# orangeai-research/Generative-Multimodal-Recommendation

Hardware: AMD Instinct MI355X
Metric: train users/sec + full-rank eval users/sec, DiffMM Amazon-baby, 1/2/4/8 MI355X (higher is better)
Workload: dtype fp32; 1 GPU; DiffMM baby-shaped synthetic: 19445 users x 7050 items, 121517 train interactions; step = one DiffMMTrainer epoch (diffusion train + graph rebuild + BPR/contrastive); global_batch=2048, eval_batch=4096, parallelism=dp1

## Files before the change

### generative-multimodal-recommendation_amd/csrc/gemm.hip

```cpp
#include <stdlib.h>

#include <type_traits>

#include "gemm_impl.h"

namespace {
using namespace gmr_gemm;

template <int BM, int BN, int WGM, int WGN, bool AKC, bool BKC, bool VEC, int MF>
__global__ void __launch_bounds__(64 * WGM * WGN) gemm_kernel(int64_t M, int64_t N, int64_t K,
                                                             const float* __restrict__ A, int64_t lda,
                                                             const float* __restrict__ B, int64_t ldb,
                                                             float* __restrict__ C, int64_t ldc, Epi epi, int tiles_n,
                                                             int64_t k_per_split, float* __restrict__ ws) {
  constexpr int NT = 64 * WGM * WGN;
  constexpr int WTM = BM / WGM, WTN = BN / WGN;
  constexpr int TM = WTM / MF, TN = WTN / MF;
  using AccT = typename std::conditional<MF == 32, floatx16, floatx4>::type;
  constexpr int NE = MF == 32 ? 16 : 4;
  using SA = Stage<BM, AKC, VEC, NT>;
  using SB = Stage<BN, BKC, VEC, NT>;
  __shared__ __attribute__((aligned(16))) float smem[2 * (SA::WORDS + SB::WORDS)];
  constexpr int STAGE_WORDS = SA::WORDS + SB::WORDS;

// ... 444 lines not shown
  int64_t tm, tn, kps;
  int xpose;
  bool x6p;
};

int default_mfma() {
  static int mf = [] {
    const char* e = getenv("GMR_GEMM_MFMA");
    return (e && atoi(e) == 16) ? 16 : 32;
  }();
  return mf;
}

bool default_x6() {
  static bool x = [] {
    const char* e = getenv("GMR_GEMM_X6");
    return !(e && atoi(e) == 0);
  }();
  return x;
}

bool default_x6_64() {
  static bool x = [] {
    const char* e = getenv("GMR_GEMM_X6_64");
    return !(e && atoi(e) == 0);
  }();
  return x;
}

bool default_glds() {
  static bool g = [] {
    const char* e = getenv("GMR_GEMM_GLDS");
    return !(e && atoi(e) == 0);
  }();
  return g;
}

int auto_splits(int64_t tm, int64_t tn, int bm, int64_t K) {
  const bool skinny = bm == 64 && (tm == 1 || tn == 1);
  const int64_t min_k = skinny ? 192 : 512;
  const int max_s = skinny ? 64 : 16;
  int s = 1;
  while (tm * tn * s < 512 && K / (s * 2) >= min_k && s < max_s) s *= 2;
  if (bm == 128) {
    const int64_t slots = 512;
    auto waves = [&](int q) { return (double)(tm * tn * q) / (double)slots; };
    auto fill = [&](int q) {
      const int64_t w = tm * tn * q;
      return (double)w / (double)(((w + slots - 1) / slots) * slots);
    };
    while ((waves(s) < 8.0 || fill(s) < 0.9) && K / (s * 2) >= min_k && s < max_s) s *= 2;
  }
  return s;
}

Plan make_plan_core(int ta, int tb, int64_t M, int64_t N, int64_t K, int tile, int split_k, bool allow_x6) {
  int mf = default_mfma();
  if (tile & GMR_GEMM_MFMA16) mf = 16;
  if (tile & GMR_GEMM_MFMA32) mf = 32;
  bool glds = default_glds();
  if (tile & GMR_GEMM_GLDS) glds = true;
  if (tile & GMR_GEMM_REGSTAGE) glds = false;
  const bool x6 = allow_x6 && ((tile & GMR_GEMM_X6) || default_x6()) &&
                  !(tile & (GMR_GEMM_F32 | GMR_GEMM_MFMA16 | GMR_GEMM_MFMA32 | GMR_GEMM_GLDS | GMR_GEMM_REGSTAGE));
  const bool x6_64 = x6 && ((tile & GMR_GEMM_X6) || default_x6_64());
  const bool x6_pipe1 = tile & GMR_GEMM_X6_PIPE1;
  tile &= ~(GMR_GEMM_MFMA16 | GMR_GEMM_MFMA32 | GMR_GEMM_GLDS | GMR_GEMM_REGSTAGE | GMR_GEMM_X6 | GMR_GEMM_F32 |
            GMR_GEMM_X6_PIPE1);
  if (tile == 0) {
    const bool tnm = ta && !tb;
    auto fill = [](int64_t tiles, int64_t slots) { return (double)tiles / (double)(((tiles + slots - 1) / slots) * slots); };
    const bool wide256 = M >= 2048 && N >= 4096 && K >= 256 && K <= 1024 &&
                         fill(((M + 255) / 256) * ((N + 255) / 256), 256) >=
                             0.92 * fill(((M + 127) / 128) * ((N + 127) / 128), 512);
    auto score = [&](int t) {
      const int64_t tm = (M + t - 1) / t, tn = (N + t - 1) / t;
      const int s = auto_splits(tm, tn, t, K);
      double pen = 1.0;
      for (int q = s; q > 1; q >>= 1) pen *= 0.95;
      return fill(tm * tn * s, t == 256 ? 256 : 512) * pen * (t == 256 ? 1.03 : 1.0);
    };
    if (!tnm && M >= 2048 && N >= 1000 && K >= 4096)
      tile = (tb || !glds) && score(256) >= score(128) ? 256 : 128;
    else if (!tnm && wide256) tile = 256;
    else if (!tnm && M * N >= (int64_t)8 << 20 && K >= 512) tile = 128;
    else if (!tnm && M * N >= (int64_t)1 << 20 && K >= 4096) tile = 128;
    else if (!ta && !tb && N <= 64 && M >= 4096 && K >= 2048) tile = 12864;
    else tile = 64;
  }
  if (x6 && tile == 64 && M * N >= ((int64_t)4 << 20) && K >= 256) tile = 128;
  if (x6 && (tile != 64 || x6_64) && tile != 12864 && !ta && tb) {
    mf = 6;
    if (tile == 256) tile = ((M + 127) / 128) * ((N + 127) / 128) >= 768 ? 128 : 256128;
  }
  Plan p;
  p.mf = mf;
  p.glds = glds && mf == 32;
  p.tile = tile;
  p.bm = tile == 256128 ? 256 : tile == 128256 || tile == 12864 ? 128 : tile;
  p.bn = tile == 256128 ? 128 : tile == 128256 ? 256 : tile == 12864 ? 64 : tile;
  p.tm = (M + p.bm - 1) / p.bm;
  p.tn = (N + p.bn - 1) / p.bn;
  int splits = split_k;
  if (splits <= 0 && mf == 6) {
    static const int64_t min_slab_env = [] {
      const char* e = getenv("GMR_X6_MIN_SLAB");
      const int v = e ? atoi(e) : 0;
      return (int64_t)(v >= 64 ? v : 0);
    }();
    const int64_t min_slab = min_slab_env ? min_slab_env : p.bm == 64 ? (x6_ring() && K <= 1024 ? K : 256) : 512;
    const int64_t slots = p.bm == 64 ? 768 : p.bm * p.bn == 128 * 128 ? 512 : 256;
    splits = 1;
    while (p.tm * p.tn * splits * 5 < slots * 4 && K / (splits * 2) >= min_slab && splits < 16) splits *= 2;
  }
  if (splits <= 0) splits = auto_splits(p.tm, p.tn, p.bm, K);
  int64_t kps = (K + splits - 1) / splits;
  kps = (kps + BK - 1) / BK * BK;
  p.splits = (int)((K + kps - 1) / kps);
  p.kps = kps;
  p.xpose = 0;
  p.x6p = mf == 6 && x6_pipe1;
  return p;
}

Plan make_plan(int ta, int tb, int64_t M, int64_t N, int64_t K, int tile, int split_k) {
  if (ta || !tb) {
    Plan q = make_plan_core(0, 1, M, N, K, tile, split_k, true);
    if (q.mf == 6 && q.bm != 64) {
      q.xpose = (ta ? 1 : 0) | (tb ? 0 : 2);
      return q;
    }
    return make_plan_core(ta, tb, M, N, K, tile, split_k, false);
  }
  return make_plan_core(ta, tb, M, N, K, tile, split_k, true);
}

struct WsLayout {
  int64_t slabs, at, bt, total, kp;
};
WsLayout ws_layout(const Plan& p, int64_t M, int64_t N, int64_t K) {
  auto r4 = [](int64_t v) { return (v + 3) / 4 * 4; };
  WsLayout w;
  w.kp = r4(K);
  const bool uses = p.splits > 1 || p.xpose;
  w.slabs = GMR_GEMM_COUNTER_WORDS;
  w.at = uses ? r4(GMR_GEMM_COUNTER_WORDS + (p.splits > 1 ? (int64_t)p.splits * M * N : 0)) : 0;
  w.bt = w.at + ((p.xpose & 1) ? r4(M * w.kp) : 0);
  w.total = w.bt + ((p.xpose & 2) ? r4(N * w.kp) : 0);
  return w;
}

}

extern "C" int32_t gmr_gemm_kernel_kind(int32_t trans_a, int32_t trans_b, int64_t M, int64_t N, int64_t K,
                                        int32_t tile, int32_t split_k, int32_t aligned) {
  if (M <= 0 || N <= 0 || K <= 0) return 0;
  const Plan p = make_plan(trans_a, trans_b, M, N, K, tile, split_k);
  if (p.mf == 6 && !aligned && p.xpose != 3)
    return make_plan_core(trans_a, trans_b, M, N, K, tile, split_k, false).mf;
  return p.mf;
}

extern "C" int64_t gmr_gemm_workspace_floats(int32_t trans_a, int32_t trans_b, int64_t M, int64_t N, int64_t K,
                                             int32_t tile, int32_t split_k) {
  if (M <= 0 || N <= 0 || K <= 0) return 0;
  const Plan p = make_plan(trans_a, trans_b, M, N, K, tile, split_k);
  int64_t need = ws_layout(p, M, N, K).total;
  if (p.mf == 6) {
    const Plan q = make_plan_core(trans_a, trans_b, M, N, K, tile, split_k, false);
    need = std::max(need, ws_layout(q, M, N, K).total);
  }
  return need;
}

extern "C" int gmr_gemm_f32(int32_t trans_a, int32_t trans_b, int64_t M, int64_t N, int64_t K, float alpha,
                            const float* A, int64_t lda, const float* B, int64_t ldb, float beta, float* C,
                            int64_t ldc, int32_t epilogue, const float* bias, const int32_t* bias_row, int64_t ld_bias,
                            const float* aux, int64_t ld_aux, const float* rowvec1, const float* rowvec2, float slope,
                            int32_t tile, int32_t split_k, float* workspace, int64_t workspace_floats, void* stream) {
  GMR_ARG(A && B && C, "null operand");
  GMR_ARG(M > 0 && N > 0 && K > 0, "empty GEMM");
  GMR_ARG(lda >= (trans_a ? M : K) && ldb >= (trans_b ? K : N) && ldc >= N, "leading dimension too small");
  GMR_ARG(epilogue >= GMR_EPI_NONE && epilogue <= GMR_EPI_SCALE_BIAS, "bad epilogue");
  GMR_ARG(epilogue != GMR_EPI_LEAKY_NORM ||
              (N == 64 && aux && rowvec1 && ld_aux >= 64 && ld_aux % 4 == 0 && ldc % 4 == 0 &&
               (((uintptr_t)aux | (uintptr_t)C) & 15) == 0),
          "GMR_EPI_LEAKY_NORM: N = 64, 16-byte aligned C and aux (the normalised rows), rowvec1 (the norms)");
  GMR_ARG(!(epilogue == GMR_EPI_POSTERIOR || epilogue == GMR_EPI_DTANH || epilogue == GMR_EPI_ROWSCALE_AUX ||
            epilogue == GMR_EPI_DRELU) || aux,
          "epilogue needs aux");
  GMR_ARG(epilogue != GMR_EPI_ROWSCALE_AUX || rowvec1, "epilogue needs rowvec1");
  {
    const int t = tile & ~(GMR_GEMM_MFMA16 | GMR_GEMM_MFMA32 | GMR_GEMM_GLDS | GMR_GEMM_REGSTAGE | GMR_GEMM_X6 |
                           GMR_GEMM_F32 | GMR_GEMM_X6_PIPE1);
    GMR_ARG(t == 0 || t == 64 || t == 128 || t == 256 || t == 256128 || t == 128256 || t == 12864,
            "tile must be 0 (auto), 64, 128, 256, 256128, 128256 or 12864 (| GMR_GEMM_MFMA16 / GMR_GEMM_MFMA32)");
  }
  Epi e;
  e.kind = epilogue;
  e.alpha = alpha;
  e.beta = beta;
  e.slope = slope;
  e.bias = bias;
  e.bias_row = bias_row;
  e.ld_bias = ld_bias;
  e.aux = aux;
  e.ld_aux = ld_aux;
  e.rv1 = rowvec1;
  e.rv2 = rowvec2;
  const bool a16 = ((uintptr_t)A % 16 == 0) && lda % 4 == 0, b16 = ((uintptr_t)B % 16 == 0) && ldb % 4 == 0;
  bool vec = a16 && b16;
  Plan pl = make_plan(trans_a, trans_b, M, N, K, tile, split_k);
  if (pl.mf == 6 && !(((pl.xpose & 1) || a16) && ((pl.xpose & 2) || b16)))
    pl = make_plan_core(trans_a, trans_b, M, N, K, tile, split_k, false);
  if ((pl.xpose & 2) && x6_inplace()) pl.xpose &= ~2;
  if (pl.xpose == 1 && !trans_b && x6_inplace() == 2) pl.xpose = 0;
  const WsLayout wl = ws_layout(pl, M, N, K);
  if (pl.xpose) {
    GMR_ARG(workspace && workspace_floats >= wl.total, "needs workspace of gmr_gemm_workspace_floats(...) floats");
    GMR_ARG(((uintptr_t)workspace & 15) == 0, "workspace must be 16-byte aligned");
    if (pl.xpose & 1) {
      x6_transpose(A, lda, K, M, workspace + wl.at, wl.kp, (hipStream_t)stream);
      GMR_LAUNCHED();
      A = workspace + wl.at;
      lda = wl.kp;
    }
    if (pl.xpose & 2) {
      x6_transpose(B, ldb, K, N, workspace + wl.bt, wl.kp, (hipStream_t)stream);
      GMR_LAUNCHED();
      B = workspace + wl.bt;
      ldb = wl.kp;
    }
    if (pl.xpose & 1) trans_a = 0;
    if (pl.xpose & 2) trans_b = 1;
    vec = (pl.xpose & 1 ? true : a16) && (pl.xpose & 2 ? true : b16);
  }
  tile = pl.tile;
  const int64_t tm = pl.tm, tn = pl.tn, kps = pl.kps;
  const int splits = pl.splits;
  GMR_ARG(tm * tn < (1ll << 31), "too many tiles");
  float* ws = nullptr;
  int* counters = nullptr;
  if (splits > 1) {
    GMR_ARG(workspace && workspace_floats >= GMR_GEMM_COUNTER_WORDS + (int64_t)splits * M * N,
            "split-K needs workspace of gmr_gemm_workspace_floats(...) floats");
    ws = workspace + GMR_GEMM_COUNTER_WORDS;
    if (pl.glds && vec && tm * tn <= GMR_GEMM_COUNTER_WORDS && inkernel_fixup() && epilogue != GMR_EPI_LEAKY_NORM)
      counters = reinterpret_cast<int*>(workspace);
  }
  GMR_ARG(epilogue != GMR_EPI_LEAKY_NORM || splits > 1, "GMR_EPI_LEAKY_NORM needs a split-K plan");
  hipStream_t st = (hipStream_t)stream;
  dim3 grid((unsigned)(tm * tn), 1, (unsigned)splits);
  const int tnp = (int)tn | (tile_group(tn) << 20);
  int lrc = 0;
  switch (tile) {
    case 256:
      lrc = launch_tile<256, 256, 4, 4>(pl.mf, pl.glds, trans_a, trans_b, vec, grid, st, M, N, K, A, lda, B, ldb, C, ldc, e, tnp, kps, ws, counters, pl.x6p);
      break;
    case 256128:
      lrc = launch_tile<256, 128, 4, 2>(pl.mf, pl.glds, trans_a, trans_b, vec, grid, st, M, N, K, A, lda, B, ldb, C, ldc, e, tnp, kps, ws, counters, pl.x6p);
      break;
    case 128256:
      lrc = launch_tile<128, 256, 2, 4>(pl.mf, pl.glds, trans_a, trans_b, vec, grid, st, M, N, K, A, lda, B, ldb, C, ldc, e, tnp, kps, ws, counters, pl.x6p);
      break;
    case 12864:
      lrc = launch_tile<128, 64, 2, 2>(pl.mf, pl.glds, trans_a, trans_b, vec, grid, st, M, N, K, A, lda, B, ldb, C, ldc, e, tnp, kps, ws, counters, pl.x6p);
      break;
    case 128:
      lrc = launch_tile<128, 128, 2, 2>(pl.mf, pl.glds, trans_a, trans_b, vec, grid, st, M, N, K, A, lda, B, ldb, C, ldc, e, tnp, kps, ws, counters, pl.x6p);
      break;
    default:
      lrc = launch_tile<64, 64, 2, 2>(pl.mf, pl.glds, trans_a, trans_b, vec, grid, st, M, N, K, A, lda, B, ldb, C, ldc, e, tnp, kps, ws, counters, pl.x6p);
  }
  GMR_ARG(lrc == 0, "no split-bf16 kernel for this tile and operand layout");
  GMR_LAUNCHED();
  if (ws && !counters && epilogue == GMR_EPI_LEAKY_NORM) {
    hipLaunchKernelGGL(splitk_reduce_leaky_norm_kernel, dim3(gmr::grid_for(M * 16, 256)), dim3(256), 0, st, M, splits,
                       ws, C, ldc, e, const_cast<float*>(aux), ld_aux, const_cast<float*>(rowvec1));
    GMR_LAUNCHED();
  } else if (ws && !counters) {
    hipLaunchKernelGGL(splitk_reduce_kernel, dim3(gmr::grid_for(M * N, 256)), dim3(256), 0, st, M, N, splits, ws, C,
                       ldc, e);
    GMR_LAUNCHED();
  }
  return GMR_OK;
}
```

### generative-multimodal-recommendation_amd/csrc/gemm_impl.h

```cpp
#pragma once
#include <type_traits>

#include "gmr_common.h"

typedef float floatx16 __attribute__((ext_vector_type(16)));
typedef float floatx4 __attribute__((ext_vector_type(4)));

namespace gmr_gemm {

constexpr int BK = 32;

struct Epi {
  int kind;
  float alpha, beta, slope;
  const float* bias;
  const int* bias_row;
  int64_t ld_bias;
  const float* aux;
  int64_t ld_aux;
  const float* rv1;
  const float* rv2;
};

__device__ __forceinline__ bool epi_reads_x(const Epi& e) {
// ... 165 lines not shown
        const float b = epi.bias ? epi.bias[n] : 0.f;
#pragma unroll
        for (int e = 0; e < NE; ++e) {
          const int64_t m = m0 + wm * WTM + i * MF + (MF == 32 ? (e & 3) + 8 * (e >> 2) + 4 * h : 4 * h + e);
          if (m < M) C[m * ldc + n] = epi_fin(epi, acc[i][j][e], b, 0.f, 0.f, 0.f);
        }
      }
    return;
  }
#pragma unroll
  for (int i = 0; i < TM; ++i)
#pragma unroll
    for (int j = 0; j < TN; ++j) {
      const int64_t n = n0 + wn * WTN + j * MF + l32;
      if (n >= N) continue;
      float bv[NE], xv[NE];
#pragma unroll
      for (int e = 0; e < NE; ++e) {
        const int64_t m = m0 + wm * WTM + i * MF + (MF == 32 ? (e & 3) + 8 * (e >> 2) + 4 * h : 4 * h + e);
        const bool ok = m < M;
        bv[e] = (epi.bias && ok) ? epi.bias[(epi.bias_row ? (int64_t)epi.bias_row[m] : 0) * epi.ld_bias + n] : 0.f;
        xv[e] = (rx && ok) ? *epi_x_ptr(epi, C, ldc, m, n) : 0.f;
      }
#pragma unroll
      for (int e = 0; e < NE; ++e) {
        const int64_t m = m0 + wm * WTM + i * MF + (MF == 32 ? (e & 3) + 8 * (e >> 2) + 4 * h : 4 * h + e);
        if (m < M) C[m * ldc + n] = epi_fin(epi, acc[i][j][e], bv[e], xv[e], epi_r1(epi, m), epi_r2(epi, m));
      }
    }
}

__device__ __forceinline__ void tile_mn(int tile, int tn_packed, int tiles_m, int& tmi, int& tni) {
  const int tiles_n = tn_packed & 0xFFFFF, G = tn_packed >> 20;
  if (G <= 1) {
    tmi = tile / tiles_n;
    tni = tile - tmi * tiles_n;
    return;
  }
  const int per = G * tiles_n, g = tile / per, first = g * G;
  const int gs = min(tiles_m - first, G), rem = tile - g * per;
  tni = rem / gs;
  tmi = first + rem - tni * gs;
}


struct EpiCtx {
  const float* xb;
  int64_t ldx;
  bool rx, pure, v_in, v_out;
};
__device__ __forceinline__ EpiCtx epi_ctx(const Epi& epi, const float* C, int64_t ldc) {
  EpiCtx c;
  c.rx = epi_reads_x(epi);
  c.pure = !c.rx && !epi.bias_row && !epi.rv1 && !epi.rv2;
  c.xb = (epi.kind == GMR_EPI_NONE || epi.kind == GMR_EPI_BIAS) ? C : epi.aux;
  c.ldx = (epi.kind == GMR_EPI_NONE || epi.kind == GMR_EPI_BIAS) ? ldc : epi.ld_aux;
  c.v_out = ldc % 4 == 0 && ((uintptr_t)C & 15) == 0;
  c.v_in = (!epi.bias || (((uintptr_t)epi.bias & 15) == 0 && (!epi.bias_row || epi.ld_bias % 4 == 0))) &&
           (!c.rx || (((uintptr_t)c.xb & 15) == 0 && c.ldx % 4 == 0));
  return c;
}
__device__ __forceinline__ void epi_store4(const Epi& epi, float* __restrict__ C, int64_t ldc, int64_t N, int64_t m,
                                           int64_t n, const float (&a4)[4], const EpiCtx& ctx) {
  const bool full = n + 3 < N;
  float b4[4] = {0.f, 0.f, 0.f, 0.f}, x4[4] = {0.f, 0.f, 0.f, 0.f};
  const float* bp = epi.bias ? epi.bias + (epi.bias_row ? (int64_t)epi.bias_row[m] * epi.ld_bias : 0) + n : nullptr;
  const float* xp = ctx.rx ? ctx.xb + m * ctx.ldx + n : nullptr;
  if (full && ctx.v_in) {
    if (bp) {
      const float4 t = *reinterpret_cast<const float4*>(bp);
      b4[0] = t.x, b4[1] = t.y, b4[2] = t.z, b4[3] = t.w;
    }
    if (xp) {
      const float4 t = *reinterpret_cast<const float4*>(xp);
      x4[0] = t.x, x4[1] = t.y, x4[2] = t.z, x4[3] = t.w;
    }
  } else {
    for (int q = 0; q < 4 && n + q < N; ++q) {
      if (bp) b4[q] = bp[q];
      if (xp) x4[q] = xp[q];
    }
  }
  const float r1 = ctx.pure ? 0.f : epi_r1(epi, m), r2 = ctx.pure ? 0.f : epi_r2(epi, m);
  float o4[4];
#pragma unroll
  for (int q = 0; q < 4; ++q) o4[q] = epi_fin(epi, a4[q], b4[q], x4[q], r1, r2);
  float* o = C + m * ldc + n;
  if (full && ctx.v_out) {
    *reinterpret_cast<float4*>(o) = make_float4(o4[0], o4[1], o4[2], o4[3]);
  } else {
    for (int q = 0; q < 4 && n + q < N; ++q) o[q] = o4[q];
  }
}

template <int BM, int BN, int WGM, int WGN, int AVAIL = 2 * (BM + BN) * BK>
__device__ __forceinline__ void gemm_epilogue_lds(const floatx16 (&acc)[BM / WGM / 32][BN / WGN / 32], float* smem,
                                                  int64_t M, int64_t N, float* __restrict__ C, int64_t ldc,
                                                  const Epi& epi, int64_t m0, int64_t n0, float* __restrict__ ws) {
  constexpr int NT = 64 * WGM * WGN;
  constexpr int WTM = BM / WGM, WTN = BN / WGN;
  constexpr int TM = WTM / 32, TN = WTN / 32;
  constexpr int HR0 = (AVAIL / BN) / 32 * 32;
  constexpr int HR = HR0 < BM ? HR0 : BM;
  constexpr int C4 = BN / 4;
  const int lane = threadIdx.x & 63;
  const int w = threadIdx.x >> 6;
  const int wm = w / WGN, wn = w % WGN;
  const int h = lane >> 5, l32 = lane & 31;
  const EpiCtx ctx = epi_ctx(epi, C, ldc);
  const bool v_out = ws ? (N % 4 == 0 && ((uintptr_t)ws & 15) == 0) : ctx.v_out;
#pragma unroll
  for (int r0 = 0; r0 < BM; r0 += HR) {
    __syncthreads();
#pragma unroll
    for (int i = 0; i < TM; ++i) {
      const int rb = wm * WTM + i * 32;
      if (rb < r0 || rb >= r0 + HR) continue;
#pragma unroll
      for (int j = 0; j < TN; ++j) {
        const int col = wn * WTN + j * 32 + l32;
#pragma unroll
        for (int e = 0; e < 16; ++e) smem[(rb - r0 + (e & 3) + 8 * (e >> 2) + 4 * h) * BN + col] = acc[i][j][e];
      }
    }
    __syncthreads();
    const int rows = BM - r0 < HR ? BM - r0 : HR;
    for (int idx = threadIdx.x; idx < rows * C4; idx += NT) {
      const int rr = idx / C4, c = (idx % C4) * 4;
      const int64_t m = m0 + r0 + rr, n = n0 + c;
      if (m >= M || n >= N) continue;
      const float4 v = *reinterpret_cast<const float4*>(smem + rr * BN + c);
      const float a4[4] = {v.x, v.y, v.z, v.w};
      const bool full = n + 3 < N;
      if (ws) {
        float* o = ws + ((int64_t)blockIdx.z * M + m) * N + n;
        if (full && v_out) {
          *reinterpret_cast<float4*>(o) = v;
        } else {
          for (int q = 0; q < 4 && n + q < N; ++q) o[q] = a4[q];
        }
        continue;
      }
      epi_store4(epi, C, ldc, N, m, n, a4, ctx);
    }
  }
}

int x6_ring();
int x6_inplace();
int x6_launch(int bm, int bn, dim3 grid, hipStream_t st, int64_t M, int64_t N, int64_t K, const float* A, int64_t lda,
              const float* B, int64_t ldb, float* C, int64_t ldc, const Epi& epi, int tiles_n, int64_t kps, float* ws,
              bool akc = true, bool bkc = true, bool pipe = false);

void x6_transpose(const float* src, int64_t ld_src, int64_t rows, int64_t cols, float* dst, int64_t ld_dst,
                  hipStream_t st);

}
```

### generative-multimodal-recommendation_amd/csrc/gemm_x6.hip

```cpp
#include <stdlib.h>

#include <type_traits>

#include "gemm_impl.h"
#include "x6_split.h"

namespace {
using namespace gmr_gemm;

typedef __bf16 bf16x8 __attribute__((ext_vector_type(8)));
typedef __bf16 bf16x4 __attribute__((ext_vector_type(4)));

__device__ __forceinline__ int x6_swz(int r) { return (r >> 2) & 3; }

__device__ __forceinline__ void split3(float x, __bf16& h, __bf16& m, __bf16& l) {
  h = (__bf16)__builtin_amdgcn_fmed3f(x, -0x1.fep127f, 0x1.fep127f);
  const float r1 = x - (float)h;
  m = (__bf16)r1;
  l = (__bf16)(r1 - (float)m);
}

template <int N, typename V>
__device__ __forceinline__ void split3n(const float* v, V& h, V& m, V& l) {
  typedef unsigned U __attribute__((ext_vector_type(N / 2)));
  U hh, mm, ll;
#pragma unroll
  for (int e = 0; e < N / 2; ++e) {
    unsigned a, b, c;
    gmr_x6::split_pair(v[2 * e], v[2 * e + 1], a, b, c);
    hh[e] = a, mm[e] = b, ll[e] = c;
  }
  h = __builtin_bit_cast(V, hh);
  m = __builtin_bit_cast(V, mm);
  l = __builtin_bit_cast(V, ll);
}

template <int R, bool KC, int NT, int N4>
__device__ __forceinline__ void x6_store(const float4 (&r)[N4], __bf16* s) {
  constexpr int PL = R * BK;
  const int t = threadIdx.x;
#pragma unroll
  for (int i = 0; i < N4; ++i) {
    const int idx = t + NT * i;
    const float v[4] = {r[i].x, r[i].y, r[i].z, r[i].w};
    if (KC) {
      const int rr = idx / (BK / 4), k4 = (idx % (BK / 4)) * 4;
      bf16x4 h, m, l;
      split3n<4>(v, h, m, l);
      const int off = rr * BK + (((k4 >> 3) ^ x6_swz(rr)) << 3) + (k4 & 7);
      *reinterpret_cast<bf16x4*>(s + off) = h;
      *reinterpret_cast<bf16x4*>(s + PL + off) = m;
      *reinterpret_cast<bf16x4*>(s + 2 * PL + off) = l;
    } else {
      const int kk = idx / (R / 4), m4 = (idx % (R / 4)) * 4;
#pragma unroll
      for (int e = 0; e < 4; ++e) {
        const int rr = m4 + e;
        const int off = rr * BK + (((kk >> 3) ^ x6_swz(rr)) << 3) + (kk & 7);
        __bf16 a, b, c;
        split3(v[e], a, b, c);
        s[off] = a;
        s[PL + off] = b;
        s[2 * PL + off] = c;
      }
    }
  }
}

template <int R, int NT>
struct KcTile {
  static constexpr int N4 = R * BK / 4 / NT;
  static_assert(N4 * NT * 4 == R * BK, "tile rows x BK must split evenly over the block");
  int off[N4];
  float4 r[N4];

  __device__ __forceinline__ void init(int64_t r0, int64_t nrows, int64_t ld) {
#pragma unroll
    for (int i = 0; i < N4; ++i) {
      const int idx = threadIdx.x + NT * i;
      const int rr = idx / (BK / 4), k4 = (idx % (BK / 4)) * 4;
      const int64_t row = min(r0 + rr, nrows - 1) - r0;
      off[i] = (int)(row * ld) + k4;
    }
  }
  __device__ __forceinline__ void load(const float* __restrict__ base) {
#pragma unroll
    for (int i = 0; i < N4; ++i) r[i] = *reinterpret_cast<const float4*>(base + off[i]);
  }
  __device__ __forceinline__ void load_tail(const float* __restrict__ base, int kleft) {
#pragma unroll
    for (int i = 0; i < N4; ++i) {
      const int k4 = ((threadIdx.x + NT * i) % (BK / 4)) * 4;
      float4 v = make_float4(0.f, 0.f, 0.f, 0.f);
      if (k4 < kleft) {
        v = *reinterpret_cast<const float4*>(base + off[i]);
        if (k4 + 1 >= kleft) v.y = 0.f;
        if (k4 + 2 >= kleft) v.z = 0.f;
        if (k4 + 3 >= kleft) v.w = 0.f;
      }
      r[i] = v;
    }
  }
};

template <int R, int NT>
struct MnTile {
  static constexpr int E = R * BK / NT;
  static_assert(E % 8 == 0 && NT % R == 0, "whole 8-k chunks of one row per thread");
  int off;
  int rr;
  int kt;
  int64_t ld;
  float v[E];

  __device__ __forceinline__ void init(int64_t r0, int64_t nrows, int64_t ld_) {
    ld = ld_;
    rr = threadIdx.x % R;
    kt = (threadIdx.x / R) * E;
    off = (int)(kt * ld + (min(r0 + rr, nrows - 1) - r0));
  }
  __device__ __forceinline__ void load(const float* __restrict__ base, int kleft) {
#pragma unroll
    for (int e = 0; e < E; ++e) v[e] = (kleft == BK || kt + e < kleft) ? base[off + e * ld] : 0.f;
  }
  __device__ __forceinline__ void store(__bf16* s) const {
    constexpr int PL = R * BK;
#pragma unroll
    for (int c = 0; c < E / 8; ++c) {
      bf16x8 h, m, l;
      split3n<8>(v + 8 * c, h, m, l);
      const int o = rr * BK + ((((kt >> 3) + c) ^ x6_swz(rr)) << 3);
      *reinterpret_cast<bf16x8*>(s + o) = h;
      *reinterpret_cast<bf16x8*>(s + PL + o) = m;
      *reinterpret_cast<bf16x8*>(s + 2 * PL + o) = l;
    }
  }
};

template <int R, int NT, int N4>
__device__ __forceinline__ void kc_fetch(float4 (&d)[N4], const KcTile<R, NT>& tl, const float* __restrict__ base,
                                         bool full, int kleft) {
  if (full) {
#pragma unroll
    for (int i = 0; i < N4; ++i) d[i] = *reinterpret_cast<const float4*>(base + tl.off[i]);
  } else {
#pragma unroll
    for (int i = 0; i < N4; ++i) {
      const int k4 = ((threadIdx.x + NT * i) % (BK / 4)) * 4;
      float4 v = make_float4(0.f, 0.f, 0.f, 0.f);
      if (k4 < kleft) {
        v = *reinterpret_cast<const float4*>(base + tl.off[i]);
        if (k4 + 1 >= kleft) v.y = 0.f;
        if (k4 + 2 >= kleft) v.z = 0.f;
        if (k4 + 3 >= kleft) v.w = 0.f;
      }
      d[i] = v;
    }
  }
}

template <int BM, int BN, int WGM, int WGN, int NBUF, int OCC, int PIPE, bool AKC = true, bool BKC = true>
__global__ void __launch_bounds__(64 * WGM * WGN, OCC) gemm_x6_kernel(int64_t M, int64_t N, int64_t K,
                                                                const float* __restrict__ A, int64_t lda,
                                                                const float* __restrict__ B, int64_t ldb,
                                                                float* __restrict__ C, int64_t ldc, Epi epi,
                                                                int tiles_n, int64_t k_per_split,
                                                                float* __restrict__ ws) {
  constexpr int NT = 64 * WGM * WGN;
  constexpr int WTM = BM / WGM, WTN = BN / WGN;
  constexpr int TM = WTM / 32, TN = WTN / 32;
  constexpr int APL = BM * BK, BPL = BN * BK;
  constexpr int STAGE = 3 * (APL + BPL);
  __shared__ __attribute__((aligned(16))) __bf16 smem[NBUF * STAGE];

  const int nwg = gridDim.x;
  const int b = blockIdx.x;
  const int xcd = b & 7, q = nwg >> 3, r = nwg & 7;
  const int tile = (xcd < r ? xcd * (q + 1) : r * (q + 1) + (xcd - r) * q) + (b >> 3);
  int tmi, tni;
  tile_mn(tile, tiles_n, (int)((M + BM - 1) / BM), tmi, tni);
  const int64_t m0 = (int64_t)tmi * BM;
  const int64_t n0 = (int64_t)tni * BN;
  const int64_t kbeg = (int64_t)blockIdx.z * k_per_split;
  const int64_t kend = min(K, kbeg + k_per_split);

  const int lane = threadIdx.x & 63;
  const int w = threadIdx.x >> 6;
  const int wm = w / WGN, wn = w % WGN;
  const int h = lane >> 5, l32 = lane & 31;

  floatx16 acc[TM][TN], sml[TM][TN];
#pragma unroll
  for (int i = 0; i < TM; ++i)
#pragma unroll
    for (int j = 0; j < TN; ++j)
#pragma unroll
      for (int e = 0; e < 16; ++e) acc[i][j][e] = sml[i][j][e] = 0.f;

  auto mstep = [&](const __bf16* a_s, int s, auto&& gap) {
    const __bf16* b_s = a_s + 3 * APL;
    bf16x8 fb[3][TN];
#pragma unroll
    for (int j = 0; j < TN; ++j) {
      const int row = wn * WTN + j * 32 + l32;
      const int off = row * BK + (((2 * s + h) ^ x6_swz(row)) << 3);
#pragma unroll
      for (int p = 0; p < 3; ++p) fb[p][j] = *reinterpret_cast<const bf16x8*>(b_s + p * BPL + off);
    }
    bf16x8 fa_[TM][3];
    auto read_a = [&](int i) {
      const int row = wm * WTM + i * 32 + l32;
      const int off = row * BK + (((2 * s + h) ^ x6_swz(row)) << 3);
#pragma unroll
      for (int p = 0; p < 3; ++p) fa_[i][p] = *reinterpret_cast<const bf16x8*>(a_s + p * APL + off);
    };
    if constexpr (PIPE == 1) {
#pragma unroll
      for (int i = 0; i < TM; ++i) read_a(i);
      __builtin_amdgcn_sched_barrier(0);
    }
#pragma unroll
    for (int i = 0; i < TM; ++i) {
      if constexpr (PIPE != 1) read_a(i);
      const bf16x8(&fa)[3] = fa_[i];
#pragma unroll
      for (int j = 0; j < TN; ++j) {
        const int g = 6 * (i * TN + j);
        sml[i][j] = __builtin_amdgcn_mfma_f32_32x32x16_bf16(fa[1], fb[1][j], sml[i][j], 0, 0, 0);
        gap(g);
        sml[i][j] = __builtin_amdgcn_mfma_f32_32x32x16_bf16(fa[0], fb[2][j], sml[i][j], 0, 0, 0);
        gap(g + 1);
        sml[i][j] = __builtin_amdgcn_mfma_f32_32x32x16_bf16(fa[2], fb[0][j], sml[i][j], 0, 0, 0);
        gap(g + 2);
        sml[i][j] = __builtin_amdgcn_mfma_f32_32x32x16_bf16(fa[0], fb[1][j], sml[i][j], 0, 0, 0);
        gap(g + 3);
        sml[i][j] = __builtin_amdgcn_mfma_f32_32x32x16_bf16(fa[1], fb[0][j], sml[i][j], 0, 0, 0);
        gap(g + 4);
        acc[i][j] = __builtin_amdgcn_mfma_f32_32x32x16_bf16(fa[0], fb[0][j], acc[i][j], 0, 0, 0);
        gap(g + 5);
      }
    }
  };

  auto nogap = [](int) {};
  static_assert((AKC && BKC) || PIPE == 0, "m- / n-contiguous operands: the PIPE 0 loop only");
  std::conditional_t<AKC, KcTile<BM, NT>, MnTile<BM, NT>> ra;
  std::conditional_t<BKC, KcTile<BN, NT>, MnTile<BN, NT>> rb;
  ra.init(m0, M, lda);
  rb.init(n0, N, ldb);
  const float* a0 = AKC ? A + m0 * lda : A + m0;
  const float* b0 = BKC ? B + n0 * ldb : B + n0;
  const int nk = kend > kbeg ? (int)((kend - kbeg + BK - 1) / BK) : 0;
  const int kl = (int)(kend - kbeg - (int64_t)(nk - 1) * BK);
  auto fetch = [&](int t) {
    const int64_t k0 = kbeg + (int64_t)t * BK;
    if constexpr (AKC && BKC) {
      if (t + 1 < nk || kl == BK) {
        ra.load(a0 + k0);
        rb.load(b0 + k0);
      } else {
        ra.load_tail(a0 + k0, kl);
        rb.load_tail(b0 + k0, kl);
      }
    } else {
      const int kleft = t + 1 < nk ? BK : kl;
      if constexpr (AKC) {
        if (kleft == BK) ra.load(a0 + k0);
        else ra.load_tail(a0 + k0, kleft);
      } else {
        ra.load(a0 + k0 * lda, kleft);
      }
      rb.load(b0 + k0 * ldb, kleft);
    }
  };
  auto store = [&](__bf16* s) {
    if constexpr (AKC) x6_store<BM, true, NT>(ra.r, s);
    else ra.store(s);
    if constexpr (BKC) x6_store<BN, true, NT>(rb.r, s + 3 * APL);
    else rb.store(s + 3 * APL);
  };
  if constexpr (PIPE == 2) {
    constexpr int PF = 4;
    constexpr int NA = KcTile<BM, NT>::N4, NB = KcTile<BN, NT>::N4;
    float4 qa[PF][NA], qb[PF][NB];
    auto fetch_slot = [&](float4 (&da)[NA], float4 (&db)[NB], int t) {
      if (t < nk) {
        const int64_t k0 = kbeg + (int64_t)t * BK;
        const bool full = t + 1 < nk || kl == BK;
        kc_fetch<BM, NT, NA>(da, ra, a0 + k0, full, kl);
        kc_fetch<BN, NT, NB>(db, rb, b0 + k0, full, kl);
      }
    };
#pragma unroll
    for (int q = 0; q < PF; ++q) fetch_slot(qa[q], qb[q], q);
    for (int t0 = 0; t0 < nk; t0 += PF) {
#pragma unroll
      for (int q = 0; q < PF; ++q) {
        const int t = t0 + q;
        if (t < nk) {
          __bf16* buf = smem + (t & 1) * STAGE;
          x6_store<BM, true, NT>(qa[q], buf);
          x6_store<BN, true, NT>(qb[q], buf + 3 * APL);
          __syncthreads();
          fetch_slot(qa[q], qb[q], t + PF);
          mstep(buf, 0, nogap);
          mstep(buf, 1, nogap);
        }
      }
    }
    __syncthreads();
  } else if constexpr (PIPE == 0) {
  int cur = 0;
  if (nk > 0) {
    fetch(0);
    store(smem);
  }
  __syncthreads();
  for (int t = 0; t < nk; ++t) {
    const bool more = t + 1 < nk;
    if (more) fetch(t + 1);
    const __bf16* a_s = smem + cur * STAGE;
    mstep(a_s, 0, nogap);
    mstep(a_s, 1, nogap);
    if constexpr (NBUF == 2) {
      if (more) store(smem + (cur ^ 1) * STAGE);
      __syncthreads();
      cur ^= 1;
    } else {
      __syncthreads();
      if (more) store(smem);
      __syncthreads();
    }
  }
  } else {
    static_assert(NBUF == 2, "the pipelined loop double-buffers LDS");
    constexpr int NA = KcTile<BM, NT>::N4, NB = KcTile<BN, NT>::N4, NF = NA + NB;
    constexpr int NM = 6 * TM * TN;
    constexpr int NPC = 6 * NF;
    constexpr int PPG = (NPC + 2 * NM - 1) / (2 * NM);
    float4 qa[NA], qb[NB];
    auto fetch_next = [&](int t) {
      fetch(min(t, nk - 1));
    };
    if (nk > 0) {
      fetch(0);
      x6_store<BM, true, NT>(ra.r, smem);
      x6_store<BN, true, NT>(rb.r, smem + 3 * APL);
      fetch_next(1);
    }
    __syncthreads();
    for (int t = 0; t < nk; ++t) {
#pragma unroll
      for (int i = 0; i < NA; ++i) qa[i] = ra.r[i];
#pragma unroll
      for (int i = 0; i < NB; ++i) qb[i] = rb.r[i];
      if (t + 2 < nk) fetch_next(t + 2);
      const __bf16* a_s = smem + (t & 1) * STAGE;
      __bf16* nxt = smem + ((t & 1) ^ 1) * STAGE;
      gmr_x6::Pair ps[2 * NF];
      unsigned lo[2 * NF];
      auto piece = [&](int c) {
        const int p = c / 3, ph = c % 3, gr = p >> 1;
        const float4 v = gr < NA ? qa[gr < NA ? gr : 0] : qb[gr < NA ? 0 : gr - NA];
        const float x0 = (p & 1) ? v.z : v.x, x1 = (p & 1) ? v.w : v.y;
        if (ph == 0) gmr_x6::split_p0(x0, x1, ps[p]);
        else if (ph == 1) gmr_x6::split_p1(x0, x1, ps[p]);
        else lo[p] = gmr_x6::split_p2(ps[p]);
        if (p & 1) {
          const bool isa = gr < NA;
          const int idx = threadIdx.x + NT * (isa ? gr : gr - NA);
          const int rr = idx / (BK / 4), k4 = (idx % (BK / 4)) * 4;
          const int off = rr * BK + (((k4 >> 3) ^ x6_swz(rr)) << 3) + (k4 & 7);
          __bf16* pl = nxt + (isa ? 0 : 3 * APL) + ph * (isa ? APL : BPL) + off;
          const uint2 w = ph == 0   ? make_uint2(ps[p - 1].h, ps[p].h)
                          : ph == 1 ? make_uint2(ps[p - 1].m, ps[p].m)
                                    : make_uint2(lo[p - 1], lo[p]);
          *reinterpret_cast<uint2*>(pl) = w;
        }
      };
      auto gap0 = [&](int g) {
#pragma unroll
        for (int c = g * PPG; c < (g + 1) * PPG; ++c)
          if (c < NPC) piece(c);
        __builtin_amdgcn_sched_barrier(0);
      };
      auto gap1 = [&](int g) { gap0(NM + g); };
      mstep(a_s, 0, gap0);
      mstep(a_s, 1, gap1);
      __syncthreads();
    }
  }

#pragma unroll
  for (int i = 0; i < TM; ++i)
#pragma unroll
    for (int j = 0; j < TN; ++j) acc[i][j] += sml[i][j];

  if (!ws && epi_reads_x(epi))
    gemm_epilogue_lds<BM, BN, WGM, WGN, NBUF * 3 * (BM + BN) * BK / 2>(acc, reinterpret_cast<float*>(smem), M, N, C,
                                                                     ldc, epi, m0, n0, ws);
  else
    gemm_epilogue<BM, BN, WGM, WGN, 32>(acc, M, N, C, ldc, epi, m0, n0, ws);
}

__global__ void __launch_bounds__(256) x6_transpose_kernel(const float* __restrict__ src, int64_t ld_src,
                                                           int64_t rows, int64_t cols, float* __restrict__ dst,
                                                           int64_t ld_dst, int64_t tiles_c) {
  __shared__ float t[64][65];
  const int64_t tr = blockIdx.x / tiles_c, tc = blockIdx.x % tiles_c;
  const int64_t r0 = tr * 64, c0 = tc * 64;
  const int x = threadIdx.x & 63, y = threadIdx.x >> 6;
#pragma unroll
  for (int i = 0; i < 16; ++i) {
    const int64_t r = r0 + y + 4 * i, c = c0 + x;
    t[y + 4 * i][x] = (r < rows && c < cols) ? src[r * ld_src + c] : 0.f;
  }
  __syncthreads();
#pragma unroll
  for (int i = 0; i < 16; ++i) {
    const int64_t c = c0 + y + 4 * i, r = r0 + x;
    if (c < cols && r < rows) dst[c * ld_dst + r] = t[x][y + 4 * i];
  }
}

}

namespace gmr_gemm {

void x6_transpose(const float* src, int64_t ld_src, int64_t rows, int64_t cols, float* dst, int64_t ld_dst,
                  hipStream_t st) {
  const int64_t tr = (rows + 63) / 64, tc = (cols + 63) / 64;
  hipLaunchKernelGGL(x6_transpose_kernel, dim3((unsigned)(tr * tc)), dim3(256), 0, st, src, ld_src, rows, cols, dst,
                     ld_dst, tc);
}

static int x6_pipe() {
  static const int v = [] {
    const char* e = getenv("GMR_GEMM_X6_PIPE");
    return e ? atoi(e) : -1;
  }();
  return v;
}

int x6_ring() {
  static const int v = [] {
    const char* e = getenv("GMR_X6_RING");
    return e ? atoi(e) : 1;
  }();
  return v;
}

static int x6_nb128() {
  static const int v = [] {
    const char* e = getenv("GMR_GEMM_X6_NB128");
    return e ? atoi(e) : 0;
  }();
  return v;
}

int x6_inplace() {
  static const int v = [] {
    const char* e = getenv("GMR_X6_INPLACE");
    return e ? atoi(e) : 0;
  }();
  return v;
}

int x6_launch(int bm, int bn, dim3 grid, hipStream_t st, int64_t M, int64_t N, int64_t K, const float* A, int64_t lda,
              const float* B, int64_t ldb, float* C, int64_t ldc, const Epi& epi, int tiles_n, int64_t kps, float* ws,
              bool akc, bool bkc, bool pipe) {
  if (x6_pipe() == 0 || x6_pipe() == 1) pipe = x6_pipe() == 1;
  if (x6_pipe() == 2) pipe = pipe || bm * bn == 256 * 128;
#define GMR_X6(BM_, BN_, WGM_, WGN_, NBUF_, OCC_)                                                                \
  {                                                                                                                \
    if (!akc || !bkc) {                                                                                            \
      if (akc)                                                                                                     \
        hipLaunchKernelGGL((gemm_x6_kernel<BM_, BN_, WGM_, WGN_, NBUF_, OCC_, 0, true, false>), grid,              \
                           dim3(64 * WGM_ * WGN_), 0, st, M, N, K, A, lda, B, ldb, C, ldc, epi, tiles_n, kps, ws); \
      else if (!bkc)                                                                                               \
        hipLaunchKernelGGL((gemm_x6_kernel<BM_, BN_, WGM_, WGN_, NBUF_, OCC_, 0, false, false>), grid,             \
                           dim3(64 * WGM_ * WGN_), 0, st, M, N, K, A, lda, B, ldb, C, ldc, epi, tiles_n, kps, ws); \
      else                                                                                                         \
        return -1;                                                                                                 \
      return 0;                                                                                                    \
    }                                                                                                              \
    if (NBUF_ == 2 && pipe)                                                                                        \
      hipLaunchKernelGGL((gemm_x6_kernel<BM_, BN_, WGM_, WGN_, NBUF_, OCC_, NBUF_ - 1>), grid, dim3(64 * WGM_ * WGN_), \
                         0, st, M, N, K, A, lda, B, ldb, C, ldc, epi, tiles_n, kps, ws);                           \
    else                                                                                                           \
      hipLaunchKernelGGL((gemm_x6_kernel<BM_, BN_, WGM_, WGN_, NBUF_, OCC_, 0>), grid, dim3(64 * WGM_ * WGN_), 0,   \
                         st, M, N, K, A, lda, B, ldb, C, ldc, epi, tiles_n, kps, ws);                              \
    return 0;                                                                                                      \
  }
  if (bm == 64 && bn == 64 && (!akc || !bkc)) return -1;
  if (bm == 64 && bn == 64 && x6_ring()) {
    hipLaunchKernelGGL((gemm_x6_kernel<64, 64, 2, 2, 2, 3, 2>), grid, dim3(256), 0, st, M, N, K, A, lda, B, ldb, C,
                       ldc, epi, tiles_n, kps, ws);
    return 0;
  }
  if (bm == 64 && bn == 64) GMR_X6(64, 64, 2, 2, 2, 3)
  if (bm == 256 && bn == 128) GMR_X6(256, 128, 4, 2, 2, 1)
  if (bm == 128 && bn == 256) GMR_X6(128, 256, 2, 4, 2, 1)
  if (bm == 128 && bn == 128) {
    const int nb = x6_nb128();
    if (nb == 2 || (pipe && akc && bkc && nb == 0)) GMR_X6(128, 128, 2, 2, 2, 1)
    if (nb == 3) GMR_X6(128, 128, 2, 2, 1, 3)
    GMR_X6(128, 128, 2, 2, 1, 2)
  }
#undef GMR_X6
  return -1;
}

}
```

### generative-multimodal-recommendation_amd/gmr/_lib.py

```python
import ctypes
import os

_HERE = os.path.dirname(os.path.abspath(__file__))
LIB_PATH = os.environ.get("GMR_HIP_LIB", os.path.join(_HERE, "libgmr_hip.so"))

P = ctypes.c_void_p
I32 = ctypes.c_int32
I64 = ctypes.c_int64
U64 = ctypes.c_uint64
F32 = ctypes.c_float
F64 = ctypes.c_double
CP = ctypes.c_char_p



class SpmmJob(ctypes.Structure):
    _fields_ = [("col", P), ("val", P), ("plan", P), ("partial", P), ("n_rows", I64), ("nnz", I64),
                ("seg_nnz", I32), ("n_blocks", I32), ("flags", I32), ("reserved", I32),
                ("x_lo", P * 4), ("ld_lo", I64 * 4), ("x_hi", P * 4), ("ld_hi", I64 * 4), ("split", I64),
                ("alpha", F32), ("beta", F32), ("y", P * 4), ("ld_y", I64 * 4)]


SIGNATURES = {
    "gmr_last_error_string": (CP, []),
    "gmr_version": (I32, []),
    "gmr_device_name": (I32, [P, I32]),
    "gmr_zero": (I32, [P, I64, P]),
    "gmr_spmm_plan_words": (I64, [I64, I64, I32]),
    "gmr_sqnorm_nparts": (I64, [I64]),
    "gmr_spmm_partial_rows": (I64, [I64, I64, I32]),
    "gmr_spmm_plan_build": (I32, [P, I64, I64, I32, P, P]),
    "gmr_spmm_plan_build_split": (I32, [P, I64, I64, I32, I64, P, P]),
    "gmr_spmm_plan_pack": (I32, [P, P, P, I64, I64, I32, P, P]),
    "gmr_spmm_plan_info": (I32, [P, P, P]),
    "gmr_event_create": (I32, [P]),
    "gmr_event_destroy": (I32, [P]),
    "gmr_stream_fork": (I32, [P, P, P]),
    "gmr_delay": (I32, [I32, P]),
    "gmr_score_f16": (I32, [I64, I64, I64, P, I64, P, I64, P, I64, P]),
    "gmr_spmm_multi_f32": (I32, [P, P, I64, I64, P, I32, I32, P, P, P, P, I64, F32, F32, P, P, P, I32, P]),
    "gmr_spmm_jobs_f32": (I32, [I32, P, P]),
    "gmr_spmm_panel_f32": (I32, [P, P, I64, I64, P, I32, I32, P, I64, F32, F32, P, I64, P, I32, P]),
    "gmr_spmm_csr_f32": (I32, [P, P, P, I64, I64, P, I32, P, I32, P, P, P, P, I64, F32, F32, P, I64, I32, P]),
    "gmr_spmm_side_plan_words": (I64, [P, I64, I64, I32]),
    "gmr_spmm_side_plan_build": (I32, [P, I64, I64, I32, P, I64]),
    "gmr_spmm_side_scratch_floats": (I64, [P]),
    "gmr_spmm_side_pack": (I32, [P, P, P, I64, I64, I64, P, P]),
    "gmr_spmm_side_pack_classes": (I32, [P, P, P, P, P, P]),
    "gmr_spmm_side_tune": (I32, [I32, I32]),
    "gmr_spmm_side_f32": (I32, [P, I32, P, P, P, P, I64, F32, F32, P, P, P, I32, P]),
    "gmr_spmm_side2_f32": (I32, [P, I32, P, P, P, P, I64, F32, F32, P, P, P, P, I32, P, I32, P]),
    "gmr_spmm_side_jobs_f32": (I32, [I32, P, P, I32, P, P, P, P, P, F32, F32, P, P, I32, P]),
    "gmr_bipartite_nnz": (I64, [I64, I64, I64, I32]),
    "gmr_bipartite_workspace_ints": (I64, [I64, I64]),
    "gmr_bipartite_symnorm_build": (I32, [I64, I64, P, P, I64, I32, F64, P, P, P, P, P]),
    "gmr_topk_to_user_csr": (I32, [I64, I32, P, I64, P, P, P]),
    "gmr_gemm_workspace_floats": (I64, [I32, I32, I64, I64, I64, I32, I32]),
    "gmr_gemm_kernel_kind": (I32, [I32, I32, I64, I64, I64, I32, I32, I32]),
    "gmr_gemm_f32": (I32, [I32, I32, I64, I64, I64, F32, P, I64, P, I64, F32, P, I64, I32, P, P, I64, P, I64, P, P,
                           F32, I32, I32, P, I64, P]),
    "gmr_split3_planes": (I32, [I64, I64, P, I64, P, I64, I64, P]),
    "gmr_dmm_combine_fwd": (I32, [I64, P, P, P, P, P, F32, P, P]),
    "gmr_dmm_final_fwd": (I32, [I64, P, P, F32, P, P, P]),
    "gmr_dmm_cl_fwd": (I32, [I64, P, P, P, P, P, P]),
    "gmr_dmm_final_bwd": (I32, [I64, P, P, P, P, F32, P, P, P, P, P]),
    "gmr_dmm_final_bwd_partials": (I64, [I64]),
    "gmr_dmm_mw_grad": (I32, [I64, P, P, P, I32, P]),
    "gmr_dmm_dg": (I32, [I64, I64, P, P, P, P]),
    "gmr_dmm_cl_bwd": (I32, [I64, P, P, P, F32, P, P, P]),
    "gmr_dmm_assemble": (I32, [I64, I64, P, P, P, P, P, F32, P, P, P]),
    "gmr_dmm_final_bwd2": (I32, [I64, P, P, P, P, F32, P, P, P, P, I32, F32, P, P, P]),
    "gmr_dmm_cl_bwd2": (I32, [I64, P, P, P, F32, P, P, I32, I32, P]),
    "gmr_dmm_assemble2": (I32, [I64, I64, P, P, P, P, P, F32, P, P, P, P, F32, P, I32, P]),
    "gmr_dmm_bpr_sqnorm": (I32, [I32, I64, P, P, P, P, P, P, F32, I64, P, P, P]),
    "gmr_dmm_loss_mw": (I32, [I64, P, F32, P, I64, F32, P, P, F32, P, P, I64, P, P, P, P]),
    "gmr_scatter_sorted_nbwd_f32": (I32, [I32, P, P, I64, P, P, I64, P, P]),
    "gmr_contrast_fused_nbwd_f32": (I32, [I32, I64, P, I64, P, I64, P, P, I64, F32, F32, P, P, I64, P, I64, P, I64, P, P,
                                          I64, P]),
    "gmr_normalize_rows_f32": (I32, [I64, I32, P, I64, P, I64, P, P]),
    "gmr_normalize_rows_bwd_f32": (I32, [I64, I32, P, I64, P, P, I64, P, I64, F32, I32, P]),
    "gmr_bpr_fwd_bwd": (I32, [I32, I64, P, P, P, P, P, P, F32, P]),
    "gmr_row_softmax_f32": (I32, [I64, I64, P, I64, F32, P, P]),
    "gmr_contrast_rows": (I32, [I32, P, P, I64, P, F32, F32, P, P, I64, P]),
    "gmr_contrast_workspace_floats": (I64, [I32, I64]),
    "gmr_contrast_fused_f32": (I32, [I32, I64, P, I64, P, I64, P, P, I64, F32, F32, P, P, I64, P, I64, P, I64, P]),
    "gmr_gather_rows_f32": (I32, [I32, I32, P, I64, P, I64, P, I64, P]),
    "gmr_scatter_sorted_f32": (I32, [I32, I32, P, P, I64, P, I64, P]),
    "gmr_sort_batch_keys": (I32, [I64, P, P, P, I32, I64, P, I64, I32, P]),
    "gmr_sum_f32": (I32, [I64, P, F32, P, I32, P]),
    "gmr_sqnorm_f32": (I32, [I64, P, F32, P, I32, P, P]),
    "gmr_sqnorm_part_f32": (I32, [I64, P, P, P]),
    "gmr_dmm_loss_total": (I32, [I64, P, F32, P, I64, F32, P, P, F32, P, P]),
    "gmr_sum_f64": (I32, [I64, P, F64, P, I32, P]),
    "gmr_colsum_f32": (I32, [I64, I64, P, I64, P, I32, P, I32, P]),
    "gmr_sample_epoch": (I32, [I64, P, P, P, P, P, I64, U64, U64, P, P, P, P, P]),
    "gmr_permutation": (I32, [I64, U64, U64, P, P]),
    "gmr_diff_sample_t": (I32, [I32, I32, U64, U64, I64, P, P]),
    "gmr_diff_qsample": (I32, [I32, I32, P, P, P, P, P, P, P, I64, P, I64, F32, I32, U64, U64, I64, P, I64, P]),
    "gmr_diff_densify": (I32, [I32, I32, P, P, P, P, I64, P]),
    "gmr_diff_time_bias": (I32, [I32, I32, P, P, P, I64, I64, P, I32, P, P, P, P]),
    "gmr_diff_loss_rows": (I32, [I32, I32, P, P, P, P, P, P, P, I64, F32, P, P, P, I32, P]),
    "gmr_vbpr_loss_fwd_bwd": (I32, [I32, I32, P, I64, P, P, P, I64, F32, P, P, P, P, P, I64, P]),
    "gmr_fill2d_f32": (I32, [I64, I64, P, I64, F32, P]),
    "gmr_transpose_f32": (I32, [I64, I64, P, I64, P, I64, P]),
    "gmr_diff_sparse_hidden": (I32, [I32, I32, P, P, P, P, I64, P, P, I64, P]),
    "gmr_diff_sparse_pre": (I32, [I32, I32, P, P, P, P, I64, P, P, I64, P, I64, P]),
    "gmr_tanh_bias_f32": (I32, [I64, I32, P, I64, P, P, I64, P]),
    "gmr_diff_sample_t_importance": (I32, [I32, I32, I32, P, P, F64, U64, U64, I64, P, P, P]),
    "gmr_diff_history_update": (I32, [I32, I32, I32, P, P, P, P, P]),
    "gmr_diff_gc_rows": (I32, [I32, P, P, P, P, I64, P, I64, F32, P, I64, P, P]),
    "gmr_diff_time_bwd": (I32, [I32, I32, I32, P, P, P, P, I64, I64, P, P, P, P, I32, P]),
    "gmr_mask_scores_f32": (I32, [I64, P, P, P, I64, F32, P]),
    "gmr_topk_rows_f32": (I32, [I64, I64, P, I64, I32, P, I64, P, P]),
    "gmr_score_topk_f32": (I32, [I64, P, P, I64, I64, P, I64, I64, P, P, F32, I32, P, I64, P, P]),
    "gmr_score_topk_x6": (I32, [I64, P, P, I64, I64, P, I64, I64, I64, P, P, F32, I32, P, I64, P, P]),
    "gmr_eval_metrics_partials": (I64, [I64]),
    "gmr_eval_metrics": (I32, [I64, P, I64, I32, P, P, I32, P, P, P, P]),
    "gmr_eval_metrics_sel": (I32, [I64, P, P, I64, I32, P, P, I32, P, P, P, P]),
    "gmr_topk_item_counts": (I32, [I64, P, I64, I32, P, I64, P, P]),
    "gmr_adam_f32": (I32, [I64, P, P, P, P, F32, F32, F32, F32, F32, F32, P]),
    "gmr_colsum_split_floats": (I64, [I64]),
    "gmr_colsum_split_f32": (I32, [I64, I64, P, I64, P, I32, P, I64, P]),
    "gmr_bn_parts_doubles": (I64, [I64]),
    "gmr_bn_fwd_f32": (I32, [I64, P, I64, I32, F32, F32, P, P, P, P, P, P, P, I32, F32, P, I64, F32, P, I64, I32, P, I64, P, P, I64, P, P]),
    "gmr_bn_bwd_f32": (I32, [I64, P, I64, P, P, P, P, I32, F32, P, I64, F32, P, I64, P, I64, P, P, P, P, P, P, P, I32, P, I64, I32, P]),
    "gmr_gr_parts": (I64, [I64]),
    "gmr_gr_content_fwd": (I32, [I64, P, P, P, P, P, P, P]),
    "gmr_gr_content_bwd": (I32, [I64, P, P, P, P, P, P, P, P, F32, P, P, P, P, P]),
    "gmr_gr_fusion_fwd": (I32, [I64, P, P, P, P, P, P, P, P, P]),
    "gmr_gr_fusion_bwd": (I32, [I64, P, P, P, P, P, P, P, P, P, P, P, P, P]),
    "gmr_mul64_f32": (I32, [I64, P, I64, P, I64, P, I64, F32, I32, P]),
    "gmr_dot64_f32": (I32, [I64, P, I64, P, I64, P, F32, P, I32, P]),
    "gmr_nce_rows_f32": (I32, [I64, P, I64, F32, P, P]),
    "gmr_nce_rows_off_f32": (I32, [I64, I64, P, I64, I64, F32, P, P]),
    "gmr_bpr_logsigmoid_f32": (I32, [I32, I64, P, P, P, P, P, P, F32, P]),
    "gmr_axpy_dev_f32": (I32, [I64, P, P, P, P]),
    "gmr_mul_f32": (I32, [I64, P, P, P, P]),
    "gmr_keep_mask_u8": (I32, [I64, F32, U64, U64, U64, P, P]),
    "gmr_csr_transpose": (I32, [I64, I64, I64, P, P, P, P, P, P, P, P, P, P]),
    "gmr_csr_drop_count": (I32, [I64, P, P, I32, P, F32, U64, U64, P, P, P]),
    "gmr_csr_drop_write": (I32, [I64, P, P, P, I32, P, F32, U64, U64, P, P, P, P]),
    "gmr_knn_symnorm_csr": (I32, [I64, I32, P, I64, P, I64, P, P, P, P, P]),
    "gmr_gen_mask": (I32, [I32, I32, I32, P, I64, P, P, I64, P, P]),
    "gmr_debias_select": (I32, [I32, I32, P, I64, P, P, I64, F32, U64, U64, P, P, I32, P, P]),
    "gmr_debias_apply": (I32, [I32, P, P, I32, P, I64, I32, P, P, I64, P]),
    "gmr_kmeans_standardize": (I32, [I64, I32, P, I64, P, P, P, I64, P, P]),
    "gmr_kmeans_pp_pick": (I32, [I64, P, U64, U64, P, P]),
    "gmr_kmeans_take_center": (I32, [I32, P, I64, P, P, I64, I32, P, P, P]),
    "gmr_kmeans_min_dist": (I32, [I64, P, P, I64, P, I32, P, I32, P]),
    "gmr_kmeans_pp_greedy": (I32, [I64, I32, P, P, I64, P, P, P, I64, I32, P, I64, I32, P, P]),
    "gmr_kmeans_parts": (I64, [I64]),
    "gmr_kmeans_assign": (I32, [I64, I32, P, I64, P, P, P, P, I64, P, P, P]),
    "gmr_kmeans_centroids": (I32, [I32, I32, P, I64, P, I64, I64, P, I64, P, P]),
    "gmr_flip_schedule": (I32, [I32, P, P, I32, I32, P, P]),
    "gmr_flip_qsample": (I32, [I32, I32, P, I64, P, I32, P, I32, F32, P, I64, U64, U64, I64, P, I64, P]),
    "gmr_flip_step": (I32, [I32, I32, P, I64, P, I32, I32, I32, P, I64, U64, U64, I64, P, I64, P, I64, P]),
    "gmr_flip_loss_rows": (I32, [I32, I32, P, I64, P, I64, P, P, I32, F32, P, I64, P, P, P]),
    "gmr_flip_total": (I32, [P, P, F32, P, P]),
    "gmr_layernorm_fwd": (I32, [I64, I32, P, I64, P, I64, P, I64, F32, P, P, F32, I32, P, I64, P, I64, P, P, P]),
    "gmr_layernorm_drop_fwd": (I32, [I64, I32, P, I64, P, I64, F32, U64, U64, U64, P, I64, F32, P, P, F32, I32, P, I64,
                                     P, I64, P, P, P]),
    "gmr_layernorm_parts_floats": (I64, [I64, I32]),
    "gmr_layernorm_bwd": (I32, [I64, I32, P, I64, P, P, P, P, I32, P, I64, P, I64, I32, P, P, P, I32, P]),
    "gmr_adaln_fwd": (I32, [I64, I32, P, I64, P, I32, P, I64, P, I64, P]),
    "gmr_adaln_bwd": (I32, [I64, I32, P, I64, P, I64, P, P, I64, P, I64, P, I64, P]),
    "gmr_dropout_f32": (I32, [I64, I32, I32, P, I64, F32, P, P, I64, U64, U64, I64, P, I64, P]),
    "gmr_time_embedding": (I32, [I32, I32, P, P]),
    "gmr_silu_f32": (I32, [I64, P, P, P, P]),
    "gmr_xattn_table_f32": (I32, [I32, I32, I32, P, P, I64, F32, P, P]),
    "gmr_decoder_layers_fwd_f32": (I32, [I64, I64, I32, I32, I32, P, P, I64, I32, F32, U64, U64, I64, I32, P, P, I32, P,
                                         I64, P]),
    "gmr_xattn_fwd_f32": (I32, [I64, I32, I32, P, P, F32, P, P, I64, U64, U64, I64, P, I64, P]),
    "gmr_xattn_bwd_workspace_floats": (I64, [I64, I32, I32]),
    "gmr_xattn_bwd_f32": (I32, [I64, I32, I32, P, I64, P, I64, P, P, F32, P, P, P, I64, P]),
    "gmr_nce_pairs_f32": (I32, [I32, I64, I64, I64, P, P, P, I64, P, I64, P]),
    "gmr_nce_combine_f32": (I32, [I32, I64, I64, I64, P, P, P, I64, P, I64, P, I64, P]),
    "gmr_frd_loss_fwd_bwd": (I32, [I32, I64, P, I64, P, I64, P, I64, P, P, P, F32, F32, P, P, P, I64, P]),
    "gmr_frd_prune_keys": (I32, [I64, P, P, U64, U64, P, P]),
    "gmr_frd_prune_workspace_ints": (I64, []),
    "gmr_frd_prune_select": (I32, [I64, I64, P, P, P, P]),
    "gmr_frd_knn_union_csr": (I32, [I64, I32, P, I64, F32, P, I64, F32, P, P, P, P, P, P, P]),
    "gmr_frd_mean_fwd": (I32, [I64, I64, I32, P, P, P, I64, P, I64, P]),
    "gmr_rf_param_floats": (I64, [I32, I32]),
    "gmr_rf_tile_rows": (I32, []),
    "gmr_rf_sample": (I32, [I64, I32, I32, I32, I32, P, I64, P, I64, P, P, I64, P]),
    "gmr_rf_act_fwd": (I32, [I64, P, P, P, P, P, F32, P, P, P, P]),
    "gmr_rf_act_parts_floats": (I64, [I64]),
    "gmr_rf_act_bwd": (I32, [I64, P, P, P, P, P, F32, P, P, P, P, P, P, P]),
    "gmr_rf_time_embed": (I32, [I64, P, P, P]),
    "gmr_rf_interp": (I32, [I64, P, I64, P, P, P, P]),
    "gmr_rf_head_fwd": (I32, [I64, P, P, P, I64, P, P, F32, P, P, P]),
    "gmr_rf_head_prior_fwd": (I32, [I64, P, P, P, I64, P, P, P, I64, F32, F32, P, P, P]),
    "gmr_rf_head_bwd": (I32, [I64, P, P, I64, P, P, P, P, P]),
    "gmr_rf_item_inputs_ws_floats": (I64, [I64]),
    "gmr_rf_item_inputs": (I32, [I64, I64, P, I64, P, I64, P, I64, P, I64, P, P]),
    "gmr_rf_view_prior_ws_floats": (I64, [I64, I64]),
    "gmr_rf_view_prior": (I32, [I64, I64, P, I64, P, I64, P, I64, P, P]),
    "gmr_rf_losses": (I32, [I64, P, I64, P, F32, P, P]),
    "gmr_rf_infonce_sampled_fwd_bwd": (I32, [I32, I64, P, I64, P, I64, I64, P, I32, P, U64, U64, U64, F32, F32, P, P,
                                             I64, P]),
    "gmr_adamw_f32": (I32, [I64, P, P, P, P, F32, F32, F32, F32, F32, F32, P]),
    "gmr_rf_randn": (I32, [I64, U64, U64, U64, P, P]),
    "gmr_rf_rand": (I32, [I64, U64, U64, U64, P, P]),
    "gmr_ld4_film_fwd": (I32, [I64, I32, P, I64, P, P, P, I64, P, I64, F32, P, I64, P, P, P]),
    "gmr_ld4_film_parts_floats": (I64, [I64, I32]),
    "gmr_ld4_film_bwd": (I32, [I64, I32, P, I64, P, P, P, P, P, I64, P, I64, P, I64, P, I64, P, I64, I32, P, P, P, I32,
                               P]),
    "gmr_ld4_gelu_drop_fwd": (I32, [I64, I32, P, I64, F32, P, P, I64, U64, U64, U64, P, I64, P]),
    "gmr_ld4_gelu_drop_bwd": (I32, [I64, I32, P, I64, P, I64, F32, P, I64, P, I64, P]),
    "gmr_ld4_add_bias": (I32, [I64, I32, P, I64, P, P, I64, P]),
    "gmr_ld4_loss_rows":(I32, [I32, I32, P, P, P, F32, P, I64, F32, P, I32, P]),
    "gmr_ld4_history_ema": (I32, [I32, I32, P, P, P, P]),
    "gmr_ld4_sample_t": (I32, [I32, I32, P, P, U64, U64, I64, P, P]),
    "gmr_ddrm_tile_rows": (I32, []),
    "gmr_ddrm_denoise_fwd": (I32, [I64, I32, I32, I64, P, I64, P, P, I64, P, P, P, P, P, I64, I32, P, I64, U64, U64,
                                   U64, P, P, P, P, P, I64, P, I64, P, I64, P, I64, P, P]),
    "gmr_ddrm_chain": (I32, [I64, I32, I32, I32, I64, P, I64, P, I64, F32, F32, P, I64, P, P, P, P, P, P, P, P, P,
                             U64, U64, U64, P, I64, P]),
    "gmr_ddrm_loss_fwd_bwd": (I32, [I32, I64, P, I64, P, P, P, P, I64, P, I64, P, P, P, F32, F32, F32, F32, P, P, P,
                                    I64, P, P, P]),
    "gmr_ddrm_input_bwd": (I32, [I64, P, P, I64, P, P, P, P, I64, P]),
    "gmr_bm3_tile_rows": (I32, []),
    "gmr_bm3_loss_fwd_bwd": (I32, [I32, I64, P, I64, P, I64, P, I64, P, P, P, I64, P, F32, F32, F32, I32, P, P, P, P,
                                   I64, U64, U64, U64, P, P, P, P, I64, P, P, I64, P, P, P]),
    "gmr_bm3_loss_reduce": (I32, [I32, P, P, I32, I32, F32, F32, F32, I64, P, P]),
    "gmr_bm3_reg_bwd": (I32, [I64, I64, P, P, I64, P, I64, P]),
    "gmr_mgcn_tile_rows": (I32, []),
    "gmr_mgcn_max_blocks": (I32, []),
    "gmr_mgcn_purify_fwd": (I32, [I64, P, I64, P, I64, P, I64, P, P, P, P, I64, P, P, I64, P, P, I64, P]),
    "gmr_mgcn_purify_bwd": (I32, [I64, P, P, I64, P, P, I64, P, I64, P, P, I64, P, I64, I32, P, I64, P, P, I64, P]),
    "gmr_mgcn_fuse_fwd": (I32, [I64, P, P, I64, P, I64, P, P, P, P, P, P, P, I64, P, P, I64, P, P, P, P, I64, P, P]),
    "gmr_mgcn_fuse_bwd": (I32, [I64, P, I64, P, P, I64, P, P, I64, P, P, P, P, I64, P, P, P, P, P, I64, P, P, I64, P,
                                I64, P, P, P, P, I64, P, I64, P]),
    "gmr_mgcn_bpr_reg_fwd_bwd": (I32, [I32, I64, P, I64, P, P, P, F32, F32, F32, P, P, I64, P]),
    "gmr_mgcn_loss_reduce": (I32, [I32, P, F32, F32, F32, F32, P, P]),
    "gmr_lat_edge_fwd": (I32, [I64, I32, I32, P, I64, P, I64, P, I64, P, I64, P, P, P, I64, P, P, P]),
    "gmr_lat_adj_fwd": (I32, [I64, I32, I32, P, P, P, I64, P, P, F32, P, P]),
    "gmr_lat_sddmm": (I32, [I64, I32, P, I64, P, I64, P, I64, I32, P, P]),
    "gmr_lat_bwd_ds": (I32, [I64, I32, I32, P, P, P, P, P, I64, P, P, P, F32, P, P]),
    "gmr_lat_bwd_da": (I32, [I64, I32, I32, P, P, P, P, P, I64, P, P, F32, P, P, P]),
    "gmr_lat_dw_reduce": (I32, [I64, P, P, P, P]),
    "gmr_lat_bwd_dn": (I32, [I64, I32, I32, P, P, I64, P, I64, P, I64, P, P, P, I64, P, I64, P]),
    "gmr_smore_tile_rows": (I32, []),
    "gmr_smore_max_blocks": (I32, []),
    "gmr_smore_spectrum_ws_floats": (I64, [I64]),
    "gmr_smore_twiddles": (I32, [P, P, P]),
    "gmr_smore_spectrum_fwd": (I32, [I64, P, I64, P, I64, P, I64, P, P, P, P, P, P, P, P, P, I64, P, I64, P, I64, P,
                                     I64, P, I64, P]),
    "gmr_smore_spectrum_bwd": (I32, [I64, P, I64, P, I64, P, I64, P, I64, P, P, P, P, P, P, I64, P, I64, I32, P, I64,
                                     P, P, I64, P, I64, P, P, P, P]),
    "gmr_smore_fuse_fwd": (I32, [I64, P, I64, P, I64, P, P, P, P, P, P, P, P, P, P, P, P, I64, F32, I32, P, I64, U64,
                                 U64, P, P, I64, P, I64, P]),
    "gmr_smore_fuse_bwd": (I32, [I64, P, I64, P, P, I64, P, I64, P, I64, F32, P, P, P, P, P, P, P, I64, P, I64, P,
                                 I64, P, I64, P]),
    "gmr_lgm_tile_rows": (I32, []),
    "gmr_lgm_max_blocks": (I32, []),
    "gmr_lgm_lat_ws_floats": (I64, [I64, I32]),
    "gmr_lgm_hyper_fwd": (I32, [I64, I64, I32, P, I64, P, I64, P, P, P, P, I64, P, P, I64, F32, F32, I32, U64, U64, P,
                                P, I64, I32, P]),
    "gmr_lgm_draws": (I32, [I64, I32, I32, U64, U64, F32, P, P, P]),
    "gmr_lgm_lat": (I32, [I64, P, I64, I32, P, P, I64, P, I64, I32, P, P]),
    "gmr_lgm_apply": (I32, [I64, P, I64, I32, P, P, I64, I32, I32, P]),
    "gmr_lgm_combine_fwd": (I32, [I64, P, I64, P, I64, P, I64, I32, P, F32, P, I64, P, P, P, I32, P]),
    "gmr_lgm_combine_bwd": (I32, [I64, P, I64, P, I64, P, P, P, F32, P, I64, P, I32, P]),
    "gmr_lgm_dh": (I32, [I64, P, P, I64, P, I32, P, I64, P, P, I64, F32, F32, P, I64, I32, P]),
    "gmr_lgm_logit_bwd": (I32, [I64, I64, I32, P, I64, P, P, P, I64, P, I64, I32, P]),
# ... 55 lines not shown
```

### generative-multimodal-recommendation_amd/gmr/denoise.py

```python
import math
import os

import numpy as np
import torch
import torch.nn as nn

from . import _lib
from . import dist
from . import kernels as K
from .abstract_recommender import r4
from .kernels import ptr, stream
from .slab import Slab


PSAMPLE_FOLD = os.environ.get("GMR_PSAMPLE_FOLD", "1") != "0"


class _Linear(nn.Module):
    def __init__(self, weight, bias):
        super().__init__()
        self.weight = weight
        self.bias = bias


class Denoiser(nn.Module):
    PARAM_NAMES = ("emb_W", "emb_b", "W1", "b1", "W2", "b2")

    def __init__(self, n_items, hidden, emb_size, device, dropout=0.5, norm=False):
        super().__init__()
        if norm:
            raise NotImplementedError("Denoise(norm=True) is not on the configured hot path")
        I, H, E = n_items, hidden, emb_size
        self.I, self.H, self.E = I, H, E
        self.ld_w1 = r4(I + E)
        self.keep_prob = 1.0 - dropout
        self.slab = Slab([("emb_W", (E, E), None), ("emb_b", (E,), None), ("W1", (H, I + E), self.ld_w1),
                          ("b1", (H,), None), ("W2", (I, H), r4(H)), ("b2", (I,), None)], device)
        self.emb_layer = _Linear(self.slab.parameter("emb_W"), self.slab.parameter("emb_b"))
        self.in_layers = nn.ModuleList([_Linear(self.slab.parameter("W1"), self.slab.parameter("b1"))])
        self.out_layers = nn.ModuleList([_Linear(self.slab.parameter("W2"), self.slab.parameter("b2"))])
        self.device = device
        self._tb = None

    def params(self):
        return [self.emb_layer.weight, self.emb_layer.bias, self.in_layers[0].weight, self.in_layers[0].bias,
                self.out_layers[0].weight, self.out_layers[0].bias]

    @torch.no_grad()
    def init_like_reference(self):
        I, H, E = self.I, self.H, self.E
        emb = nn.Linear(E, E)
        lin_in = nn.Linear(I + E, H)
        lin_out = nn.Linear(H, I)
        nn.Dropout(1.0 - self.keep_prob)
        for lay in (lin_in, lin_out, emb):
            size = lay.weight.size()
            lay.weight.data.normal_(0.0, float(np.sqrt(2.0 / (size[0] + size[1]))))
            lay.bias.data.normal_(0.0, 0.001)
        self.slab.load("emb_W", emb.weight)
        self.slab.load("emb_b", emb.bias)
        self.slab.load("W1", lin_in.weight)
        self.slab.load("b1", lin_in.bias)
        self.slab.load("W2", lin_out.weight)
        self.slab.load("b2", lin_out.bias)

    def time_bias(self, T):
        if self._tb is None or self._tb[0].shape[0] != T:
            self._tb = (torch.empty((T, self.H), device=self.device), torch.empty((T, self.E), device=self.device),
                        torch.empty((T, self.E), device=self.device))
        EB, temb, emb = self._tb
        s = self.slab
        _lib.call("gmr_diff_time_bias", T, self.E, ptr(s.view("emb_W")), ptr(s.view("emb_b")), ptr(s.view("W1")),
                  self.ld_w1, self.I, ptr(s.view("b1")), self.H, ptr(EB), ptr(temb), ptr(emb), stream())
        return self._tb

    def W1x(self):
        return self.slab.view("W1")[:, :self.I]

    def refresh_w1t(self):
        if getattr(self, "_w1t", None) is None:
            self._w1t = torch.empty((self.I, r4(self.H)), device=self.device)[:, :self.H]
        _lib.call("gmr_transpose_f32", self.H, self.I, ptr(self.slab.view("W1")), self.ld_w1, ptr(self._w1t),
                  self._w1t.stride(0), stream())
        if PSAMPLE_FOLD:
            self.refresh_fold()
        return self._w1t

    def refresh_fold(self):
        H = self.H
        if getattr(self, "_fold", None) is None:
            self._fold = (torch.empty((H, r4(H)), device=self.device)[:, :H],
                          torch.empty((1, r4(H)), device=self.device)[:, :H])
        P, v = self._fold
        K.gemm(self.W1x(), self.slab.view("W2"), P)
        K.gemm(self.slab.view("b2")[None, :], self.W1x(), v, trans_b=True)
        return self._fold

    def p_sample_fold(self, users, user_ptr, user_items, EB, c1, c2, x, a, h):
        T = len(c1)
        if c2[0] != 0.0:
            raise ValueError("p_sample_fold needs c2[0] == 0 (the posterior mean at t = 0 is the x0 prediction)")
        P, v = self._fold
        B, H = users.numel(), self.H
        _lib.call("gmr_diff_sparse_pre", B, H, ptr(users), ptr(user_ptr), ptr(user_items), ptr(self._w1t),
                  self._w1t.stride(0), ptr(EB[T - 1]), ptr(a), a.stride(0), ptr(h), h.stride(0), stream())
        for i in range(T - 1, 0, -1):
            K.gemm(h, P, a, trans_b=True, epi=K.EPI_POSTERIOR, bias=v[0], aux=a, slope=c1[i], beta=c2[i])
            _lib.call("gmr_tanh_bias_f32", B, H, ptr(a), a.stride(0), ptr(EB[i - 1]), ptr(h), h.stride(0), stream())
        return self.posterior_step(h, x, c1[0], 0.0)

    def hidden_sparse(self, users, user_ptr, user_items, h, eb_row):
        _lib.call("gmr_diff_sparse_hidden", users.numel(), self.H, ptr(users), ptr(user_ptr), ptr(user_items),
                  ptr(self._w1t), self._w1t.stride(0), ptr(eb_row), ptr(h), h.stride(0), stream())
        return h

    def hidden(self, x, h, EB, t_rows=None, t_const=None):
        if t_rows is not None:
            K.gemm(x, self.W1x(), h, trans_b=True, epi=K.EPI_BIAS_TANH, bias=EB, bias_row=t_rows, ld_bias=self.H)
        else:
            K.gemm(x, self.W1x(), h, trans_b=True, epi=K.EPI_BIAS_TANH, bias=EB[t_const], ld_bias=0)
        return h

    def output(self, h, out):
        K.gemm(h, self.slab.view("W2"), out, trans_b=True, epi=K.EPI_BIAS, bias=self.slab.view("b2"))
        return out

    def posterior_step(self, h, x, c1, c2):
        if c2 == 0.0:
            K.gemm(h, self.slab.view("W2"), x, trans_b=True, epi=K.EPI_SCALE_BIAS, bias=self.slab.view("b2"),
                   slope=c1)
        else:
            K.gemm(h, self.slab.view("W2"), x, trans_b=True, epi=K.EPI_POSTERIOR, bias=self.slab.view("b2"), aux=x,
                   slope=c1, beta=c2)
        return x

    def slab_head_words(self):
        return self.slab.offsets["W2"]

    def backward(self, x_in, h, dout, dpre, t_rows, T, S, early_reduce=False):
        s = self.slab
        I = self.I
        K.gemm(dout, h, s.gview("W2"), trans_a=True)
        K.colsum(dout, s.gview("b2"))
        if early_reduce:
            self.early_handle = dist.all_reduce_start(s.grad[self.slab_head_words():])
        K.gemm(dout, s.view("W2"), dpre, epi=K.EPI_DTANH, aux=h)
        K.gemm(dpre, x_in, s.gview("W1")[:, :I], trans_a=True)
        K.colsum(dpre, S, group=t_rows, n_groups=T)
        EB, temb, emb = self._tb
        _lib.call("gmr_diff_time_bwd", T, self.E, self.H, ptr(S), ptr(temb), ptr(emb), ptr(s.view("W1")), self.ld_w1,
                  I, ptr(s.gview("W1")), ptr(s.gview("b1")), ptr(s.gview("emb_W")), ptr(s.gview("emb_b")), 0,
                  stream())
```

### generative-multimodal-recommendation_amd/gmr/diffmm.py

```python
import os

import numpy as np
import torch
import torch.nn as nn

from . import _lib
from . import dist
from . import kernels as K
from .abstract_recommender import GeneralRecommender, config_seed
from . import denoise as dn
from .denoise import Denoiser
from .kernels import ptr, stream
from .slab import Slab

FUSE_FWD, FUSE_BWD_CL, FUSE_BWD3, FUSE_UI_T = 1, 2, 4, 8
BWD_EARLY = os.environ.get("GMR_BWD_EARLY", "1") != "0"
SPMM_FUSE = int(os.environ.get("GMR_SPMM_FUSE", str(FUSE_FWD | FUSE_BWD3)))
REBUILD_CHUNK = int(os.environ.get("GMR_REBUILD_CHUNK", "32768"))
EARLY_REDUCE = os.environ.get("GMR_DP_EARLY_REDUCE", "1") != "0"


def diffmm_tables(noise_scale, noise_min, noise_max, steps):
    var = np.linspace(noise_scale * noise_min, noise_scale * noise_max, steps, dtype=np.float64)
    ab = 1.0 - var
# ... 401 lines not shown
    def getItemEmbeds(self):
        return self.iEmbeds

    def getUserEmbeds(self):
        return self.uEmbeds

    def getImageFeats(self):
        w = self._work(1)
        self._project(w)
        return w["F"][:, :64]

    def getTextFeats(self):
        w = self._work(1)
        self._project(w)
        return w["F"][:, 64:]

    def optim_slabs(self):
        return [self.rec_slab]

    def extra_state(self):
        out = {"counters": {"rebuilds": self._rebuilds, "step": self._step}}
        for n in ("image_UI_matrix", "text_UI_matrix"):
            g = getattr(self, n)
            if g is not None:
                out[n] = {"rowptr": g.rowptr.cpu(), "col": g.col.cpu(), "val": g.val.cpu()}
                t = self._ui_T.get(id(g))
                if t is not None:
                    out[n + "_T"] = {"rowptr": t.rowptr.cpu(), "col": t.col.cpu(), "val": t.val.cpu()}
        return out

    def load_extra_state(self, st):
        def csr(d):
            if d is None:
                return None
            dev = self.device
            return K.CSR(d["rowptr"].to(dev), d["col"].to(dev), d["val"].to(dev), symmetric=False,
                         class_split=self.n_users, side=True)
        gi, gt = csr(st.get("image_UI_matrix")), csr(st.get("text_UI_matrix"))
        if gi is not None and gt is not None:
            self.set_ui_matrices(gi, gt, csr(st.get("image_UI_matrix_T")), csr(st.get("text_UI_matrix_T")))
        c = st.get("counters") or {}
        self._rebuilds = int(c.get("rebuilds", self._rebuilds))
        self._step = int(c.get("step", self._step))

    def grad_view(self, name):
        s, U = self.rec_slab, self.n_users
        if name == "uEmbeds":
            return s.gview("E0")[:U]
        if name == "iEmbeds":
            return s.gview("E0")[U:]
        return s.gview(name)

    def calculate_loss(self, interaction):
        users, pos, neg = (interaction[i].to(torch.int32).contiguous() for i in range(3))
        params = [getattr(self, n) for n in self.REC_PARAMS]
        for p in params:
            p.grad = None
        return _RecLoss.apply(self, users, pos, neg, *params)

    @torch.no_grad()
    def forward_embeddings(self):
        w = self._work(1)
        emb = self._forward_mm(w, with_cl=False)
        return emb[:self.n_users], emb[self.n_users:]

    @torch.no_grad()
    def full_sort_predict(self, interaction):
        user = interaction[0].to(torch.int32)
        usr, itm = self.forward_embeddings()
        E = user.numel()
        ub = torch.empty((E, 64), device=self.device)
        K.gather_rows(usr, user, ub)
        scores = torch.empty((E, self.n_items), device=self.device)
        K.gemm(ub, itm, scores, trans_b=True)
        return scores

    @torch.no_grad()
    def topk_from_embeddings(self, usr, itm, users_i32, mask_rows, mask_cols, k, out_idx, scores_buf, out_val=None):
        E = users_i32.numel()
        ub = scores_buf.new_empty((E, 64))
        K.gather_rows(usr, users_i32, ub)
        sc = scores_buf[:E, :self.n_items]
        K.gemm(ub, itm, sc, trans_b=True)
        K.mask_scores(sc, mask_rows, mask_cols)
        K.topk_rows(sc, k, out_idx, out_val)
        return out_idx

    def _dwork(self, B, slot=0):
        if self._dw is None:
            self._dw = {}
        cur = self._dw.get(slot)
        if cur is not None and cur["B"] >= B:
            return cur
        I, dev = self.n_items, self.device
        H = self.denoise_model_image.H
        Ip = (I + 3) // 4 * 4
        f = lambda *s, dt=torch.float32: torch.empty(s, dtype=dt, device=dev)
        self._dw[slot] = {"B": B, "x": f(B, Ip), "h": f(B, H), "out": f(B, Ip), "dpre": f(B, H), "Z": f(B, 64),
                          "Gc": f(B, 64), "S": f(self.steps, H), "t": f(B, dt=torch.int32),
                          "mse": f(B, dt=torch.float64), "diff": f(B, dt=torch.float64),
                          "gc": f(B, dt=torch.float64), "a": f(B, (H + 3) // 4 * 4)[:, :H],
                          "users": torch.arange(self.n_users, dtype=torch.int32, device=dev)}
        return self._dw[slot]

    def diffusion_step(self, den, batch_users, feats, item_embeds, step, noise=None, keep=None, t=None,
                       norm_rows=None, slot=0, row0=0, early_reduce=False):
        B = batch_users.numel()
        nr = float(norm_rows or B)
        w = self._dwork(B, slot)
        I, T = self.n_items, self.steps
        x, h, out, Z = w["x"][:B], w["h"][:B], w["out"][:B], w["Z"][:B]
        tt = w["t"][:B]
        if t is None:
            _lib.call("gmr_diff_sample_t", B, T, self.seed, step, row0, ptr(tt), stream())
        else:
            tt.copy_(t)
        EB, _, _ = den.time_bias(T)
        _lib.call("gmr_diff_qsample", B, I, ptr(batch_users), ptr(self.user_ptr), ptr(self.user_items), ptr(tt),
                  ptr(self._tab_dev["sqrt_ac"]), ptr(self._tab_dev["sqrt_1mac"]), ptr(noise),
                  noise.stride(0) if noise is not None else 0, ptr(keep), keep.stride(0) if keep is not None else 0,
                  den.keep_prob, 1, self.seed, step, row0, ptr(x), x.stride(0), stream())
        xi = x[:, :I]
        den.hidden(xi, h, EB, t_rows=tt)
        o = out[:, :I]
        den.output(h, o)
        K.gemm(o, feats, Z)
        _lib.call("gmr_diff_loss_rows", B, I, ptr(batch_users), ptr(self.user_ptr), ptr(self.user_items), ptr(tt),
                  ptr(self._w_dev), None, ptr(o), o.stride(0), 1.0 / nr, ptr(w["mse"]), ptr(w["diff"]), None, 1,
                  stream())
        gsc = self.e_loss * 2.0 / (64.0 * nr)
        _lib.call("gmr_diff_gc_rows", B, ptr(batch_users), ptr(self.user_ptr), ptr(self.user_items),
                  ptr(item_embeds), item_embeds.stride(0), ptr(Z), 64, gsc, ptr(w["Gc"]), 64, ptr(w["gc"]), stream())
        K.gemm(w["Gc"][:B], feats, o, trans_b=True, beta=1.0)
        den.backward(xi, h, o, w["dpre"][:B], tt, T, w["S"], early_reduce=early_reduce)
        return w["diff"][:B], w["gc"][:B]

    @torch.no_grad()
    def p_sample_topk(self, den, users_lo, users_hi, out_topk, k, x_out=None, w1t_fresh=False, slot=0):
        B = users_hi - users_lo
        w = self._dwork(B, slot)
        I, T = self.n_items, self.steps
        assert B <= w["B"]
        x, h = w["x"][:B], w["h"][:B]
        users = w["users"][users_lo:users_hi]
        if not dn.PSAMPLE_FOLD:
            _lib.call("gmr_diff_densify", B, I, ptr(users), ptr(self.user_ptr), ptr(self.user_items), ptr(x),
                      x.stride(0), stream())
        EB, _, _ = den.time_bias(T)
        if not w1t_fresh:
            den.refresh_w1t()
        xi = x[:, :I]
        c1 = [float(np.float32(c)) for c in self.tables["c1"]]
        c2 = [float(np.float32(c)) for c in self.tables["c2"]]
        if dn.PSAMPLE_FOLD:
            den.p_sample_fold(users, self.user_ptr, self.user_items, EB, c1, c2, xi, w["a"][:B], h)
        for i in reversed(range(T)) if not dn.PSAMPLE_FOLD else ():
            if i == T - 1:
                den.hidden_sparse(users, self.user_ptr, self.user_items, h, EB[i])
            else:
                den.hidden(xi, h, EB, t_const=i)
            den.posterior_step(h, xi, float(np.float32(self.tables["c1"][i])), float(np.float32(self.tables["c2"][i])))
        if x_out is not None:
            x_out.copy_(xi)
        if out_topk is not None:
            K.topk_rows(xi, k, out_topk[users_lo:users_hi])
        return xi

    @torch.no_grad()
    def rebuild_ui_graphs(self, chunk=None):
        U, I, k = self.n_users, self.n_items, self.rebuild_k
        dev = self.device
        chunk = chunk or REBUILD_CHUNK
        lo_r, hi_r, size = dist.padded_shard(U)
        W = dist.world()
        topks = [torch.zeros((W * size, k), dtype=torch.int32, device=dev) for _ in range(2)]
        uptr = torch.empty(U + 1, dtype=torch.int32, device=dev)
        uitems = torch.empty(U * k, dtype=torch.int32, device=dev)
        dens = (self.denoise_model_image, self.denoise_model_text)

        def sample(j):
            dens[j].refresh_w1t()
            for lo in range(lo_r, hi_r, chunk):
                self.p_sample_topk(dens[j], lo, min(hi_r, lo + chunk), topks[j], k, w1t_fresh=True, slot=j)

        st = self._streams
        with st.on(1):
            sample(1)
        sample(0)
        early = W == 1
        graphs = [None, None]

        def build(j):
            topk = topks[j]
            dist.all_gather_rows_(topk, size)
            K.topk_to_user_csr(topk[:U], uptr, uitems)
            g = K.bipartite_symnorm(U, I, uptr, uitems, self_loops=True, deg_eps=0.0)
            if self.keepRate != 1:
                st_id = 6000 + 2 * self._rebuilds + j
                graphs[j] = (K.csr_drop_edges(g, self.keepRate, seed=self.seed, step=st_id),
                             K.csr_drop_edges(g, self.keepRate, seed=self.seed, step=st_id, transposed=True))
            else:
                graphs[j] = (g, None)

        if early:
            build(0)
        st.join(1)
        if not early:
            build(0)
        build(1)
        self._rebuilds += 1
        self.set_ui_matrices(graphs[0][0], graphs[1][0], graphs[0][1], graphs[1][1])
```

### generative-multimodal-recommendation_amd/gmr/kernels.py

```python
import ctypes
import os

import torch

from . import _lib

EPI_NONE, EPI_BIAS, EPI_BIAS_TANH, EPI_LEAKY, EPI_POSTERIOR, EPI_DTANH, EPI_ROWSCALE_AUX, EPI_BIAS_RELU, EPI_DRELU = range(9)
EPI_LEAKY_NORM = 9
EPI_SCALE_BIAS = 10

_ws = {}

_probe = None
_probe_every = 1
_probe_count = 0


def probe_begin(tags, every=1):
    global _probe, _probe_every, _probe_count
    _probe = {t: [] for t in tags}
    _probe_every, _probe_count = max(1, int(every)), 0


def probe_end():
# ... 408 lines not shown
        if o.shape != (a.n_rows, 64):
            raise ValueError(f"output block shape {tuple(o.shape)} != ({a.n_rows}, 64)")
    PArr, LArr = ctypes.c_void_p * 4, ctypes.c_int64 * 4
    lo = PArr(*[b[0].data_ptr() for b in blocks] + [0] * (4 - nb))
    ldl = LArr(*[_ld(b[0]) for b in blocks] + [0] * (4 - nb))
    if split is None:
        split, hi, ldh = a.n_cols, lo, ldl
    else:
        hi = PArr(*[b[1].data_ptr() for b in blocks] + [0] * (4 - nb))
        ldh = LArr(*[_ld(b[1]) for b in blocks] + [0] * (4 - nb))
    ys = PArr(*[o.data_ptr() for o in outs] + [0] * (4 - nb))
    ldy = LArr(*[_ld(o) for o in outs] + [0] * (4 - nb))
    if a.side is not None:
        a._side_call(nb, lo, ldl, hi, ldh, split, alpha, beta, ys, ldy, partial)
        return outs
    with _Probe("spmm", (a.nnz, a.n_rows, a.n_cols, nb, beta != 0.0)):
        _lib.call("gmr_spmm_multi_f32", ptr(a.col), ptr(a.val), a.n_rows, a.nnz, ptr(a.plan), a.seg_nnz, nb, lo, ldl,
                  hi, ldh, split, float(alpha), float(beta), ys, ldy, ptr(a.partial if partial is None else partial),
                  a.flags, stream())
    return outs


SIDE_JOBS = os.environ.get("GMR_SPMM_SIDE_JOBS", "1") != "0"


def _side_jobs(jobs, alpha, beta):
    n, nb = len(jobs), len(jobs[0][2])
    PA, LA = ctypes.c_void_p * (4 * n), ctypes.c_int64 * (4 * n)
    plans, scr = (ctypes.c_void_p * n)(), (ctypes.c_void_p * n)()
    lo, hi, ys = PA(), PA(), PA()
    ldl, ldh, ldy = LA(), LA(), LA()
    splits = (ctypes.c_int64 * n)()
    key = []
    for q, (a, outs, blocks, split, partial) in enumerate(jobs):
        if isinstance(outs, torch.Tensor):
            outs = [outs[:, 64 * b:64 * (b + 1)] for b in range(nb)]
        if len(outs) != nb or any(o.shape != (a.n_rows, 64) for o in outs):
            raise ValueError("one n_rows x 64 output per block")
        plans[q] = a.side[0].data_ptr()
        scr[q] = (a.partial if partial is None else partial).data_ptr()
        splits[q] = a.n_cols if split is None else int(split)
        for b in range(nb):
            lo[4 * q + b], ldl[4 * q + b] = blocks[b][0].data_ptr(), _ld(blocks[b][0])
            src_hi = blocks[b][1] if split is not None else blocks[b][0]
            hi[4 * q + b], ldh[4 * q + b] = src_hi.data_ptr(), _ld(src_hi)
            ys[4 * q + b], ldy[4 * q + b] = outs[b].data_ptr(), _ld(outs[b])
        key.append((a.nnz, a.n_rows, a.n_cols, nb, beta != 0.0))
    with _Probe("spmm", ("side_jobs",) + tuple(key)):
        _lib.call("gmr_spmm_side_jobs_f32", n, plans, scr, nb, lo, ldl, hi, ldh, splits, float(alpha), float(beta), ys,
                  ldy, jobs[0][0].side_wpx[nb], stream())


def spmm_jobs(jobs, alpha=1.0, beta=0.0):
    n = len(jobs)
    if not 1 <= n <= 4:
        raise ValueError("1 to 4 jobs")
    if any(j[0].side is not None for j in jobs):
        lane = [j for j in jobs if j[0].side is None]
        side = [j for j in jobs if j[0].side is not None]
        if SIDE_JOBS and len(side) > 1 and len({len(j[2]) for j in side}) == 1 and \
                len({j[0].side_wpx[len(j[2])] for j in side}) == 1:
            _side_jobs(side, alpha, beta)
        else:
            for a, outs, blocks, split, partial in side:
                if isinstance(outs, torch.Tensor):
                    outs = [outs[:, 64 * b:64 * (b + 1)] for b in range(len(blocks))]
                spmm_multi(a, outs, blocks, split=split, alpha=alpha, beta=beta, partial=partial)
        if lane:
            spmm_jobs(lane, alpha=alpha, beta=beta)
        return
    arr = (_lib.SpmmJob * n)()
    for q, (a, outs, blocks, split, partial) in enumerate(jobs):
        nb = len(blocks)
        if nb not in (1, 2, 4):
            raise ValueError("1, 2 or 4 blocks of 64 columns")
        if isinstance(outs, torch.Tensor):
            if outs.shape != (a.n_rows, 64 * nb):
                raise ValueError(f"out shape {tuple(outs.shape)} != ({a.n_rows}, {64 * nb})")
            outs = [outs[:, 64 * b:64 * (b + 1)] for b in range(nb)]
        if len(outs) != nb or any(o.shape != (a.n_rows, 64) for o in outs):
            raise ValueError("one n_rows x 64 output per block")
        for b in blocks:
            if b[0].shape[1] != 64 or (split is not None and b[1].shape[1] != 64):
                raise ValueError("each block is 64 columns wide")
        j = arr[q]
        j.col, j.val, j.plan = ptr(a.col), ptr(a.val), ptr(a.plan)
        j.partial = ptr(a.partial if partial is None else partial)
        j.n_rows, j.nnz, j.seg_nnz, j.n_blocks, j.flags = a.n_rows, a.nnz, a.seg_nnz, nb, a.flags
        for b in range(nb):
            j.x_lo[b], j.ld_lo[b] = blocks[b][0].data_ptr(), _ld(blocks[b][0])
            if split is not None:
                j.x_hi[b], j.ld_hi[b] = blocks[b][1].data_ptr(), _ld(blocks[b][1])
            j.y[b], j.ld_y[b] = outs[b].data_ptr(), _ld(outs[b])
        j.split = a.n_cols if split is None else split
        j.alpha, j.beta = float(alpha), float(beta)
    key = tuple((a.nnz, a.n_rows, a.n_cols, len(bl), beta != 0.0) for a, _, bl, _, _ in jobs)
    with _Probe("spmm", ("jobs",) + key):
        _lib.call("gmr_spmm_jobs_f32", n, ctypes.cast(arr, ctypes.c_void_p), stream())


def spmm_panel(a, out, x_panel, nb, alpha=1.0, beta=0.0, partial=None):
    W = 32 if nb == 4 else 16
    if x_panel.shape != (64 * nb // W, a.n_cols, W) or not x_panel.is_contiguous():
        raise ValueError(f"x_panel must be a contiguous ({64 * nb // W}, {a.n_cols}, {W}) panel stack")
    if out.shape[0] != a.n_rows or out.shape[1] != 64 * nb:
        raise ValueError("out shape")
    with _Probe("spmm", (a.nnz, a.n_rows, a.n_cols, nb, beta != 0.0)):
        _lib.call("gmr_spmm_panel_f32", ptr(a.col), ptr(a.val), a.n_rows, a.nnz, ptr(a.plan), a.seg_nnz, nb,
                  ptr(x_panel), a.n_cols, float(alpha), float(beta), ptr(out), _ld(out),
                  ptr(a.partial if partial is None else partial), a.flags, stream())
    return out


def bipartite_symnorm(n_users, n_items, user_ptr, user_items, self_loops, deg_eps, seg_nnz=None):
    lib = _lib.load()
    dev = user_ptr.device
    n_ui = user_items.numel()
    nnz = lib.gmr_bipartite_nnz(n_users, n_items, n_ui, int(self_loops))
    N = n_users + n_items
    rowptr = torch.empty(N + 1, dtype=torch.int32, device=dev)
    col = torch.empty(max(nnz, 1), dtype=torch.int32, device=dev)
    val = torch.empty(max(nnz, 1), dtype=torch.float32, device=dev)
    ws = torch.empty(lib.gmr_bipartite_workspace_ints(n_users, n_items), dtype=torch.int32, device=dev)
    _lib.call("gmr_bipartite_symnorm_build", n_users, n_items, ptr(user_ptr), ptr(user_items), n_ui,
              int(self_loops), float(deg_eps), ptr(ws), ptr(rowptr), ptr(col), ptr(val), stream())
    return CSR(rowptr, col[:nnz], val[:nnz], seg_nnz=seg_nnz, class_split=n_users, side=True)


def topk_to_user_csr(topk, user_ptr, user_items):
    U, k = topk.shape
    _lib.call("gmr_topk_to_user_csr", U, k, ptr(topk), _ld(topk), ptr(user_ptr), ptr(user_items), stream())


def normalize_rows(x, y, nrm=None):
    n, cols = x.shape
    _lib.call("gmr_normalize_rows_f32", n, cols, ptr(x), _ld(x), ptr(y), _ld(y), ptr(nrm), stream())
    return y


def normalize_rows_bwd(y, nrm, dy, dx, slope=1.0, accumulate=False):
    n, cols = y.shape
    _lib.call("gmr_normalize_rows_bwd_f32", n, cols, ptr(y), _ld(y), ptr(nrm), ptr(dy), _ld(dy), ptr(dx), _ld(dx),
              float(slope), int(accumulate), stream())
    return dx


def topk_rows(scores, k, out_idx, out_val=None):
    n, m = scores.shape
    _lib.call("gmr_topk_rows_f32", n, m, ptr(scores), _ld(scores), int(k), ptr(out_idx), _ld(out_idx), ptr(out_val),
              stream())
    return out_idx


EVAL_X6 = os.environ.get("GMR_EVAL_X6", "0") != "0"
_item_planes = {}


def _planes_of(itm):
    key = (itm.data_ptr(), itm._version, tuple(itm.shape), _ld(itm), itm.device)
    hit = _item_planes.get("key")
    if hit is not None and hit[0] == key:
        return hit[1]
    pl = Planes(itm.shape[0], itm.shape[1], itm.device).load(itm)
    _item_planes["key"] = (key, pl)
    return pl


def score_topk(usr, itm, users, mask_ptr, mask_cols, k, out_idx, out_val=None, fill=-1e10):
    n = users.numel() if users is not None else out_idx.shape[0]
    if out_idx.shape[0] < n or mask_ptr.numel() < n + 1 or mask_ptr.dtype != torch.int64:
        raise ValueError("score_topk: out_idx / mask_ptr (int64, n + 1) too small for the rows")
    if n == 0:
        return out_idx
    if EVAL_X6 and itm.shape[1] == 64 and usr.shape[1] == 64:
        pl = _planes_of(itm)
        _lib.call("gmr_score_topk_x6", n, ptr(users), ptr(usr), _ld(usr), itm.shape[0], pl.ptr(), pl.ld, pl.ps, 64,
                  ptr(mask_ptr), ptr(mask_cols), float(fill), int(k), ptr(out_idx), _ld(out_idx), ptr(out_val),
                  stream())
        return out_idx
    _lib.call("gmr_score_topk_f32", n, ptr(users), ptr(usr), _ld(usr), itm.shape[0], ptr(itm), _ld(itm), itm.shape[1],
              ptr(mask_ptr), ptr(mask_cols), float(fill), int(k), ptr(out_idx), _ld(out_idx), ptr(out_val), stream())
    return out_idx


def mask_scores(scores, rows, cols, fill=-1e10):
    _lib.call("gmr_mask_scores_f32", rows.numel(), ptr(rows), ptr(cols), ptr(scores), _ld(scores), float(fill),
              stream())


def contrast_workspace(B, n, device, tag):
    return workspace(int(_lib.load().gmr_contrast_workspace_floats(B, n)), device, tag=tag)


def contrast_fused(P, T, CLN, nodes, node_off, inv_temp, coef, loss, contrib, dT, ws):
    B, n = (P.shape[0] if P is not None else nodes.numel()), T.shape[0]
    with _Probe("infonce", (B, n)):
        _lib.call("gmr_contrast_fused_f32", B, n, ptr(P), _ld(P) if P is not None else _ld(CLN), ptr(T), _ld(T),
                  ptr(CLN), ptr(nodes), node_off,
                  float(inv_temp), float(coef), ptr(loss), ptr(contrib), _ld(contrib), ptr(dT), _ld(dT), ptr(ws),
                  ws.numel(), stream())


def colsum(x, out, group=None, n_groups=1, accumulate=False):
    rows, cols = x.shape
    if group is None and cols <= 2048 and rows >= 1024:
        ws = workspace(32 * cols, x.device, tag="colsum")
        _lib.call("gmr_colsum_split_f32", rows, cols, ptr(x), _ld(x), ptr(out), int(accumulate), ptr(ws), ws.numel(),
                  stream())
        return out
    _lib.call("gmr_colsum_f32", rows, cols, ptr(x), _ld(x), ptr(group), n_groups, ptr(out), int(accumulate),
              stream())
    return out


def gather_rows(src, idx, out, off=0):
    B = idx.numel()
    _lib.call("gmr_gather_rows_f32", B, out.shape[1], ptr(src), _ld(src), ptr(idx), off, ptr(out), _ld(out),
              stream())
    return out


def adam(param, grad, m, v, lr, beta1, beta2, eps, weight_decay, step):
    bc1 = 1.0 - beta1 ** step
    bc2 = 1.0 - beta2 ** step
    _lib.call("gmr_adam_f32", param.numel(), ptr(param), ptr(grad), ptr(m), ptr(v), float(beta1), float(beta2),
              float(eps), float(weight_decay), float(lr / bc1), float(bc2 ** 0.5), stream())


def eval_metrics(topk, pos_ptr, pos_items, ks, partials, out_sums):
    n, K = topk.shape
    ks_t = ks
    _lib.call("gmr_eval_metrics", n, ptr(topk), _ld(topk), K, ptr(pos_ptr), ptr(pos_items), ks_t.numel(), ptr(ks_t),
              ptr(partials), ptr(out_sums), stream())


def user_item_csr(n_users, n_items, user_ptr, user_items):
    val = torch.ones(max(user_items.numel(), 1), dtype=torch.float32, device=user_ptr.device)[:user_items.numel()]
    return CSR(user_ptr, user_items, val, n_cols=n_items, symmetric=False)


def csr_transpose(a):
    dev = a.rowptr.device
    nc = a.n_cols
    trp = torch.empty(nc + 1, dtype=torch.int32, device=dev)
    n = max(a.nnz, 1)
    tcol = torch.empty(n, dtype=torch.int32, device=dev)
    tval = torch.empty(n, dtype=torch.float32, device=dev)
    scol = torch.empty(n, dtype=torch.int32, device=dev)
    sval = torch.empty(n, dtype=torch.float32, device=dev)
    ws = torch.empty(2 * nc, dtype=torch.int32, device=dev)
    _lib.call("gmr_csr_transpose", a.n_rows, nc, a.nnz, ptr(a.rowptr), ptr(a.col), ptr(a.val), ptr(ws), ptr(trp),
              ptr(tcol), ptr(tval), ptr(scol), ptr(sval), stream())
    return CSR(trp, tcol[:a.nnz], tval[:a.nnz], n_cols=a.n_rows, symmetric=False,
               class_split=a.class_split if a.n_rows == a.n_cols else 0, side=a.side is not None)


def csr_drop_edges(a, keep_rate, seed=0, step=0, keep=None, transposed=False):
    dev = a.rowptr.device
    orp = torch.empty(a.n_rows + 1, dtype=torch.int32, device=dev)
    ws = torch.empty(a.n_rows, dtype=torch.int32, device=dev)
    _lib.call("gmr_csr_drop_count", a.n_rows, ptr(a.rowptr), ptr(a.col), int(transposed), ptr(keep), float(keep_rate),
              int(seed), int(step), ptr(ws), ptr(orp), stream())
    nnz = int(orp[-1].item())
    ocol = torch.empty(max(nnz, 1), dtype=torch.int32, device=dev)
    oval = torch.empty(max(nnz, 1), dtype=torch.float32, device=dev)
    _lib.call("gmr_csr_drop_write", a.n_rows, ptr(a.rowptr), ptr(a.col), ptr(a.val), int(transposed), ptr(keep),
              float(keep_rate), int(seed), int(step), ptr(orp), ptr(ocol), ptr(oval), stream())
    return CSR(orp, ocol[:nnz], oval[:nnz], n_cols=a.n_cols, symmetric=False, class_split=a.class_split,
               side=a.side is not None)


def knn_graph(feat, k):
    n, d = feat.shape
    dev = feat.device
    fn = torch.empty((n, d), dtype=torch.float32, device=dev)
    normalize_rows(feat, fn)
    sim = torch.empty((n, (n + 3) // 4 * 4), dtype=torch.float32, device=dev)[:, :n]
    gemm(fn, fn, sim, trans_b=True)
    ti = torch.empty((n, k), dtype=torch.int32, device=dev)
    tv = torch.empty((n, k), dtype=torch.float32, device=dev)
    topk_rows(sim, k, ti, tv)
    del sim
    rp = torch.empty(n + 1, dtype=torch.int32, device=dev)
    col = torch.empty(n * k, dtype=torch.int32, device=dev)
    val = torch.empty(n * k, dtype=torch.float32, device=dev)
    dis = torch.empty(n, dtype=torch.float32, device=dev)
    _lib.call("gmr_knn_symnorm_csr", n, k, ptr(ti), k, ptr(tv), k, ptr(dis), ptr(rp), ptr(col), ptr(val), stream())
    return CSR(rp, col, val, n_cols=n, symmetric=False)
```

### include/gmr.h

```cpp
#ifndef GMR_H_
#define GMR_H_

#include <stdint.h>

#ifdef __cplusplus
extern "C" {
#endif

#define GMR_ABI_VERSION 2
#define GMR_OK 0
#define GMR_ERR_ARG (-1000)

#define GMR_EPI_NONE 0
#define GMR_EPI_BIAS 1
#define GMR_EPI_BIAS_TANH 2
#define GMR_EPI_LEAKY 3
#define GMR_EPI_POSTERIOR 4
#define GMR_EPI_DTANH 5
#define GMR_EPI_ROWSCALE_AUX 6
#define GMR_EPI_BIAS_RELU 7
#define GMR_GEMM_COUNTER_WORDS 16384
#define GMR_GEMM_GLDS (1 << 22)
#define GMR_GEMM_REGSTAGE (1 << 23)
#define GMR_GEMM_MFMA16 (1 << 24)
// ... 79 lines not shown
                     const int32_t* plan, int32_t seg_nnz, float* partial, int32_t n_blocks,
                     const float* const* x_lo, const int64_t* ld_lo, const float* const* x_hi, const int64_t* ld_hi,
                     int64_t split, float alpha, float beta, float* y, int64_t ldy, int32_t flags, void* stream);

int gmr_score_f16(int64_t E, int64_t I, int64_t d, const float* A, int64_t lda, const float* B, int64_t ldb,
                  float* C, int64_t ldc, void* stream);

int64_t gmr_bipartite_nnz(int64_t n_users, int64_t n_items, int64_t n_user_items, int32_t self_loops);
int64_t gmr_bipartite_workspace_ints(int64_t n_users, int64_t n_items);
int gmr_bipartite_symnorm_build(int64_t n_users, int64_t n_items, const int32_t* user_ptr, const int32_t* user_items,
                                int64_t n_user_items, int32_t self_loops, double deg_eps, int32_t* workspace,
                                int32_t* rowptr, int32_t* col, float* val, void* stream);
int gmr_topk_to_user_csr(int64_t n_users, int32_t k, const int32_t* topk, int64_t ld, int32_t* user_ptr,
                         int32_t* user_items, void* stream);

int32_t gmr_gemm_kernel_kind(int32_t trans_a, int32_t trans_b, int64_t M, int64_t N, int64_t K, int32_t tile,
                             int32_t split_k, int32_t aligned);
int64_t gmr_gemm_workspace_floats(int32_t trans_a, int32_t trans_b, int64_t M, int64_t N, int64_t K, int32_t tile,
                                  int32_t split_k);
int gmr_gemm_f32(int32_t trans_a, int32_t trans_b, int64_t M, int64_t N, int64_t K, float alpha, const float* A,
                 int64_t lda, const float* B, int64_t ldb, float beta, float* C, int64_t ldc, int32_t epilogue,
                 const float* bias, const int32_t* bias_row, int64_t ld_bias, const float* aux, int64_t ld_aux,
                 const float* rowvec1, const float* rowvec2, float slope, int32_t tile, int32_t split_k,
                 float* workspace, int64_t workspace_floats, void* stream);

int gmr_split3_planes(int64_t rows, int64_t cols, const float* src, int64_t ld_src, uint16_t* dst, int64_t ld_dst,
                      int64_t plane_stride, void* stream);

int gmr_dmm_combine_fwd(int64_t n, float* G, const float* H, const float* Qi, const float* Qt, const float* mw,
                        float lam, float* M, void* stream);
int gmr_dmm_final_fwd(int64_t n, const float* M, const float* L, float ris, float* Emb, float* nrm, void* stream);
int gmr_dmm_cl_fwd(int64_t n, const float* Qi, const float* Qt, const float* K2, float* CLN, float* nrm,
                   void* stream);
int gmr_dmm_final_bwd(int64_t n, const float* dEmb, const float* T1, const float* M, const float* nrmM, float ris,
                      const float* E, const float* mw, float* dE, float* partials, void* stream);
int64_t gmr_dmm_final_bwd_partials(int64_t n);
int gmr_dmm_mw_grad(int64_t nparts, const float* partials, const float* mw, float* dmw, int32_t accumulate,
                    void* stream);
int gmr_dmm_dg(int64_t n, int64_t U, const float* dE, const float* T2, float* dG, void* stream);
int gmr_dmm_cl_bwd(int64_t n, const float* dK, const float* T, const float* dE, float lam, float* Ri, float* Rt,
                   void* stream);
int gmr_dmm_assemble(int64_t n, int64_t U, const float* T2, const float* T3, const float* Ri, const float* Rt,
                     const float* E0, float reg2, float* dE0, float* dNF, void* stream);
int gmr_dmm_final_bwd2(int64_t n, float* dEmb, const float* T1, const float* M, const float* nrmM, float ris,
                       const float* E, const float* mw, float* dE, float* partials, int32_t clear, float lam, float* Ri,
                       float* Rt, void* stream);
int gmr_dmm_cl_bwd2(int64_t n, float* dK, const float* T, const float* dE, float lam, float* Ri, float* Rt,
                    int32_t clear, int32_t left, void* stream);
int gmr_dmm_assemble2(int64_t n, int64_t U, const float* T2, const float* T3, const float* Ri, const float* Rt,
                      const float* E0, float reg2, float* dE0, float* dNF, const float* NF, const float* nrmF,
                      float slope, float* dK_clear, int32_t t3u_from_t2, void* stream);
int gmr_dmm_bpr_sqnorm(int32_t B, int64_t U, const float* Emb, const int32_t* users, const int32_t* pos,
                       const int32_t* neg, float* loss, float* contrib, float inv_norm, int64_t n_sq, const float* x,
                       double* sq_parts, void* stream);
int gmr_dmm_loss_mw(int64_t B, const float* loss_bpr, float inv_nr, const double* parts, int64_t nparts,
                    float reg_scale, const float* loss_cu, const float* loss_ci, float ssl_scale, float* out,
                    float* acc, int64_t n_mw_parts, const float* mw_parts, const float* mw, float* dmw, void* stream);

int gmr_normalize_rows_f32(int64_t n, int32_t cols, const float* x, int64_t ldx, float* y, int64_t ldy, float* nrm,
                           void* stream);
int gmr_normalize_rows_bwd_f32(int64_t n, int32_t cols, const float* y, int64_t ldy, const float* nrm, const float* dy,
                               int64_t lddy, float* dx, int64_t lddx, float slope, int32_t accumulate, void* stream);

int gmr_bpr_fwd_bwd(int32_t B, int64_t U, const float* Emb, const int32_t* users, const int32_t* pos,
                    const int32_t* neg, float* loss, float* contrib, float inv_norm, void* stream);
int gmr_vbpr_loss_fwd_bwd(int32_t B, int32_t D, const float* table, int64_t ldt, const int32_t* users,
                          const int32_t* pos, const int32_t* neg, int64_t item_off, float reg_weight, float* x_ws,
                          double* sq_ws, float* coef_ws, float* loss, float* contrib, int64_t ldc, void* stream);
int gmr_fill2d_f32(int64_t rows, int64_t cols, float* p, int64_t ld, float value, void* stream);
int gmr_row_softmax_f32(int64_t rows, int64_t cols, float* L, int64_t ld, float coef, float* lse, void* stream);
int gmr_contrast_rows(int32_t B, const float* CLN, const int32_t* nodes, int64_t node_off, const float* lse,
                      float inv_temp, float coef, float* loss, float* contrib, int64_t ld_contrib, void* stream);
int64_t gmr_contrast_workspace_floats(int32_t B, int64_t n);
int gmr_contrast_fused_f32(int32_t B, int64_t n, const float* P, int64_t ldp, const float* T, int64_t ldt,
                           const float* CLN, const int32_t* nodes, int64_t node_off, float inv_temp, float coef,
                           float* loss, float* contrib, int64_t ld_contrib, float* dT, int64_t ld_dt, float* workspace,
                           int64_t workspace_floats, void* stream);
int gmr_contrast_fused_nbwd_f32(int32_t B, int64_t n, const float* P, int64_t ldp, const float* T, int64_t ldt,
                                const float* CLN, const int32_t* nodes, int64_t node_off, float inv_temp, float coef,
                                float* loss, float* contrib, int64_t ld_contrib, float* dT, int64_t ld_dt,
                                const float* y, int64_t ldy, const float* nrm, float* workspace,
                                int64_t workspace_floats, void* stream);
int gmr_gather_rows_f32(int32_t B, int32_t cols, const float* src, int64_t lds, const int32_t* idx, int64_t off,
                        float* out, int64_t ldo, void* stream);
int gmr_scatter_sorted_f32(int32_t n, int32_t cols, const uint64_t* plan, const float* contrib, int64_t ldc,
                           float* dst, int64_t ldd, void* stream);
int gmr_scatter_sorted_nbwd_f32(int32_t n, const uint64_t* plan, const float* contrib, int64_t ldc, const float* y,
                                const float* nrm, int64_t n_nodes, float* dK, void* stream);
int gmr_sort_batch_keys(int64_t n_batches, const int32_t* keys, const int64_t* offsets, const int32_t* key_add,
                        int32_t n_keysets, int64_t key_stride, uint64_t* out, int64_t out_stride, int32_t pow2,
                        void* stream);
int gmr_sum_f32(int64_t n, const float* x, float scale, float* out, int32_t accumulate, void* stream);
#define GMR_SQNORM_PARTS 1024
int gmr_sqnorm_f32(int64_t n, const float* x, float scale, float* out, int32_t accumulate, double* workspace,
                   void* stream);
int64_t gmr_sqnorm_nparts(int64_t n);
int gmr_sqnorm_part_f32(int64_t n, const float* x, double* workspace, void* stream);
int gmr_dmm_loss_total(int64_t B, const float* loss_bpr, float inv_nr, const double* parts, int64_t nparts,
                       float reg_scale, const float* loss_cu, const float* loss_ci, float ssl_scale, float* out,
                       void* stream);
int gmr_sum_f64(int64_t n, const double* x, double scale, double* out, int32_t accumulate, void* stream);
int gmr_colsum_f32(int64_t rows, int64_t cols, const float* x, int64_t ld, const int32_t* group, int32_t n_groups,
                   float* out, int32_t accumulate, void* stream);

int64_t gmr_colsum_split_floats(int64_t cols);
int gmr_colsum_split_f32(int64_t rows, int64_t cols, const float* x, int64_t ld, float* out, int32_t accumulate,
                         float* workspace, int64_t workspace_floats, void* stream);

int gmr_sample_epoch(int64_t n_inter, const int32_t* inter_user, const int32_t* inter_item, const int32_t* user_rowptr,
                     const int32_t* user_items, const int32_t* all_items, int64_t n_all_items, uint64_t seed,
                     uint64_t epoch, int32_t* out_users, int32_t* out_pos, int32_t* out_neg, int32_t* n_fallback,
                     void* stream);
int gmr_permutation(int64_t n, uint64_t seed, uint64_t epoch, int32_t* out, void* stream);

int gmr_diff_sample_t(int32_t B, int32_t T, uint64_t seed, uint64_t step, int64_t row0, int32_t* t, void* stream);
int gmr_diff_qsample(int32_t B, int32_t I, const int32_t* users, const int32_t* user_ptr, const int32_t* user_items,
                     const int32_t* t, const float* sqrt_ac, const float* sqrt_1mac, const float* noise,
                     int64_t ld_noise, const float* keep, int64_t ld_keep, float keep_prob, int32_t dropout,
                     uint64_t seed, uint64_t step, int64_t row0, float* x, int64_t ldx, void* stream);
int gmr_diff_densify(int32_t B, int32_t I, const int32_t* users, const int32_t* user_ptr, const int32_t* user_items,
                     float* x, int64_t ldx, void* stream);
int gmr_diff_time_bias(int32_t T, int32_t E, const float* emb_W, const float* emb_b, const float* W1, int64_t ld_w1,
                       int64_t col_off, const float* b1, int32_t H, float* EB, float* temb_out, float* emb_out,
                       void* stream);
int gmr_diff_loss_rows(int32_t B, int32_t I, const int32_t* users, const int32_t* user_ptr, const int32_t* user_items,
                       const int32_t* t, const double* wtab, const float* pt, float* out, int64_t ld, float grad_scale,
                       double* mse_out, double* diff_out, double* loss_out, int32_t write_grad, void* stream);
int gmr_transpose_f32(int64_t rows, int64_t cols, const float* in, int64_t ldi, float* out, int64_t ldo,
                      void* stream);
int gmr_diff_sparse_hidden(int32_t B, int32_t H, const int32_t* users, const int32_t* user_ptr,
                           const int32_t* user_items, const float* W1T, int64_t ldw, const float* eb, float* h,
                           int64_t ldh, void* stream);
int gmr_diff_sparse_pre(int32_t B, int32_t H, const int32_t* users, const int32_t* user_ptr, const int32_t* user_items,
                        const float* W1T, int64_t ldw, const float* eb, float* a, int64_t lda, float* h, int64_t ldh,
                        void* stream);
int gmr_tanh_bias_f32(int64_t rows, int32_t cols, const float* a, int64_t lda, const float* bias, float* h,
                      int64_t ldh, void* stream);
int gmr_diff_sample_t_importance(int32_t B, int32_t T, int32_t hist_len, const double* hist, const int32_t* count,
                                 double uniform_prob, uint64_t seed, uint64_t step, int64_t row0, int32_t* t,
                                 float* pt, void* stream);
int gmr_diff_history_update(int32_t B, int32_t T, int32_t hist_len, const int32_t* t, const double* loss,
                            double* hist, int32_t* count, void* stream);
int gmr_diff_gc_rows(int32_t B, const int32_t* users, const int32_t* user_ptr, const int32_t* user_items,
                     const float* item_embeds, int64_t ld_ie, const float* Z, int64_t ldz, float gscale, float* G,
                     int64_t ldg, double* gc_out, void* stream);
int gmr_diff_time_bwd(int32_t T, int32_t E, int32_t H, const float* S, const float* temb, const float* emb,
                      const float* W1, int64_t ld_w1, int64_t col_off, float* dW1, float* db1, float* d_emb_W,
                      float* d_emb_b, int32_t accumulate, void* stream);

int gmr_mask_scores_f32(int64_t n, const int32_t* rows, const int32_t* cols, float* scores, int64_t ld, float fill,
                        void* stream);
int gmr_topk_rows_f32(int64_t n_rows, int64_t n_cols, const float* scores, int64_t ld, int32_t k, int32_t* out_idx,
                      int64_t ld_idx, float* out_val, void* stream);
int gmr_score_topk_f32(int64_t n_rows, const int32_t* users, const float* user_table, int64_t ld_user, int64_t n_items,
                       const float* item_table, int64_t ld_item, int64_t dim, const int64_t* mask_ptr,
                       const int32_t* mask_cols, float fill, int32_t k, int32_t* out_idx, int64_t ld_idx,
                       float* out_val, void* stream);
int gmr_score_topk_x6(int64_t n_rows, const int32_t* users, const float* user_table, int64_t ld_user, int64_t n_items,
                      const uint16_t* item_planes, int64_t ld_plane, int64_t plane_stride, int64_t dim,
                      const int64_t* mask_ptr, const int32_t* mask_cols, float fill, int32_t k, int32_t* out_idx,
                      int64_t ld_idx, float* out_val, void* stream);
int64_t gmr_eval_metrics_partials(int64_t n_users);
int gmr_eval_metrics(int64_t n_users, const int32_t* topk, int64_t ld_topk, int32_t K, const int64_t* pos_ptr,
                     const int32_t* pos_items, int32_t n_ks, const int32_t* ks, double* partials, double* out_sums,
                     void* stream);
int gmr_eval_metrics_sel(int64_t n_sel, const int32_t* sel, const int32_t* topk, int64_t ld_topk, int32_t K,
                         const int64_t* pos_ptr, const int32_t* pos_items, int32_t n_ks, const int32_t* ks,
                         double* partials, double* out_sums, void* stream);
int gmr_topk_item_counts(int64_t n_users, const int32_t* topk, int64_t ld_topk, int32_t n_ks, const int32_t* ks,
                         int64_t n_items, int32_t* counts, void* stream);

int64_t gmr_bn_parts_doubles(int64_t rows);
int gmr_bn_fwd_f32(int64_t rows, const float* z, int64_t ldz, int32_t train, float eps, float momentum, float* run_mean,
                   float* run_var, double* parts, float* mean, float* invstd, const float* w, const float* b,
                   int32_t act, float slope, const uint8_t* keep, int64_t ld_keep, float keep_scale, float* y,
                   int64_t ldy, int32_t post, const float* aux, int64_t ld_aux, const float* rs, float* out2,
                   int64_t ld2, float* rowdot, void* stream);
int gmr_bn_bwd_f32(int64_t rows, const float* z, int64_t ldz, const float* mean, const float* invstd, const float* w,
                   const float* b, int32_t act, float slope, const uint8_t* keep, int64_t ld_keep, float keep_scale,
                   const float* dy, int64_t lddy, const float* mul, int64_t ld_mul, const float* da, const float* v,
                   double* parts, float* sums, float* dw, float* db, float* dv, int32_t accumulate_params, float* dz,
                   int64_t lddz, int32_t accumulate_dz, void* stream);
int64_t gmr_gr_parts(int64_t n);
int gmr_gr_content_fwd(int64_t n, const float* E, const float* A1, const float* A2, const float* ow, const float* gw,
                       float* C, void* stream);
int gmr_gr_content_bwd(int64_t n, const float* E, const float* A1, const float* A2, const float* dC, const float* T1,
                       const float* T2, const float* ow, const float* gw, float reg2, double* parts, float* dE,
                       float* dow, float* dgw, void* stream);
int gmr_gr_fusion_fwd(int64_t n, const float* IMG, const float* TXT, const float* aI, const float* aT,
                      const float* PI, const float* PT, float* SIDE, float* alpha, void* stream);
int gmr_gr_fusion_bwd(int64_t n, const float* IMG, const float* TXT, const float* alpha, const float* PI,
                      const float* PT, const float* dSIDE, float* dIMG, float* dTXT, float* daI, float* daT,
                      float* dPI, float* dPT, void* stream);
int gmr_mul64_f32(int64_t rows, const float* a, int64_t lda, const float* b, int64_t ldb, float* out, int64_t ldo,
                  float scale, int32_t accumulate, void* stream);
int gmr_dot64_f32(int64_t rows, const float* a, int64_t lda, const float* b, int64_t ldb, double* parts, float scale,
                  float* out, int32_t accumulate, void* stream);
int gmr_nce_rows_f32(int64_t B, float* L, int64_t ld, float coef, float* loss, void* stream);
int gmr_nce_rows_off_f32(int64_t rows, int64_t cols, float* L, int64_t ld, int64_t diag_off, float coef, float* loss,
                         void* stream);
int gmr_nce_pairs_f32(int32_t nterms, int64_t B, int64_t Bg, int64_t row0, const int32_t* i1, const int32_t* i2,
                      const float* nv, int64_t tab, float* cln, int64_t ct, void* stream);
int gmr_nce_combine_f32(int32_t nterms, int64_t B, int64_t Bg, int64_t row0, const int32_t* i1, const int32_t* i2,
                        const float* contrib, int64_t ct, const float* dT, int64_t dts, float* g, int64_t tab,
                        void* stream);
int gmr_bpr_logsigmoid_f32(int32_t B, int64_t U, const float* C, const int32_t* users, const int32_t* pos,
                           const int32_t* neg, float* loss, float* contrib, float inv_norm, void* stream);

int gmr_axpy_dev_f32(int64_t n, const float* alpha, const float* x, float* y, void* stream);
int gmr_mul_f32(int64_t n, const float* a, const float* b, float* out, void* stream);
int gmr_keep_mask_u8(int64_t n, float p_keep, uint64_t seed, uint64_t step, uint64_t ctr0, uint8_t* out, void* stream);

int gmr_csr_transpose(int64_t n_rows, int64_t n_cols, int64_t nnz, const int32_t* rowptr, const int32_t* col,
                      const float* val, int32_t* workspace, int32_t* t_rowptr, int32_t* t_col, float* t_val,
                      int32_t* stage_col, float* stage_val, void* stream);
int gmr_csr_drop_count(int64_t n_rows, const int32_t* rowptr, const int32_t* col, int32_t transposed,
                       const uint8_t* keep, float keep_rate, uint64_t seed, uint64_t step, int32_t* workspace,
                       int32_t* out_rowptr, void* stream);
int gmr_csr_drop_write(int64_t n_rows, const int32_t* rowptr, const int32_t* col, const float* val,
                       int32_t transposed, const uint8_t* keep, float keep_rate, uint64_t seed, uint64_t step,
                       const int32_t* out_rowptr, int32_t* out_col, float* out_val, void* stream);
int gmr_knn_symnorm_csr(int64_t n, int32_t k, const int32_t* topi, int64_t ldi, const float* topv, int64_t ldv,
                        float* dis_ws, int32_t* rowptr, int32_t* col, float* val, void* stream);
int gmr_gen_mask(int32_t B, int32_t I, int32_t k, const int32_t* topi, int64_t ldt, const float* x0, const float* xs,
                 int64_t ld, float* den, void* stream);
int gmr_debias_select(int32_t B, int32_t k, const int32_t* topi, int64_t ldt, const float* x0, const float* xs,
                      int64_t ld, float ratio, uint64_t seed, uint64_t step, uint64_t* keys_ws ,
                      int32_t* picks, int32_t max_picks, int32_t* n_picks, void* stream);
int gmr_debias_apply(int32_t type, const int32_t* picks, const int32_t* n_picks, int32_t max_picks, const float* x0,
                     int64_t ld0, int32_t I, const int32_t* labels, float* den, int64_t ldd, void* stream);
int gmr_kmeans_standardize(int64_t n, int32_t d, const float* X, int64_t ldx, float* mean, float* scale, float* Y,
                           int64_t ldy, float* sq, void* stream);
int gmr_kmeans_pp_pick(int64_t n, const float* mind, uint64_t seed, uint64_t step, int32_t* out, void* stream);
int gmr_kmeans_take_center(int32_t d, const float* X, int64_t ldx, const int32_t* idx, float* C, int64_t ldc,
                           int32_t j, const float* xsq, float* csq, void* stream);
int gmr_kmeans_pp_greedy(int64_t n, int32_t L, const float* xsq, const float* dots, int64_t ldd, const float* ccsq,
                         float* mind, const float* Cc, int64_t ldcc, int32_t d, float* C, int64_t ldc, int32_t j,
                         float* csq, void* stream);
int gmr_kmeans_min_dist(int64_t n, const float* xsq, const float* dots, int64_t ld_dots, const float* csq, int32_t j,
                        float* mind, int32_t first, void* stream);
int64_t gmr_kmeans_parts(int64_t n);
int gmr_kmeans_assign(int64_t n, int32_t k, const float* dots, int64_t ldd, const float* csq, const float* xsq,
                      int32_t* label, float* onehot_t, int64_t ldo, int32_t* changed, double* inertia_parts,
                      void* stream);
int gmr_kmeans_centroids(int32_t k, int32_t d, const float* sums, int64_t lds, const float* onehot_t, int64_t ldo,
                         int64_t n, float* C, int64_t ldc, float* csq, void* stream);

int gmr_flip_schedule(int32_t B, const int32_t* users, const int32_t* user_ptr, int32_t I, int32_t T, float* tables,
                      void* stream);
int gmr_flip_qsample(int32_t B, int32_t I, const float* x0, int64_t ld0, const int32_t* t, int32_t t_const,
                     const float* tables, int32_t T, float temp, const uint8_t* flip, int64_t ld_flip, uint64_t seed,
                     uint64_t step, int64_t row0, float* xt, int64_t ldt, void* stream);
int gmr_flip_step(int32_t B, int32_t I, const float* z, int64_t ldz, const float* tables, int32_t T, int32_t qi,
                  int32_t last,
                  const uint8_t* draws, int64_t ldd, uint64_t seed, uint64_t step, int64_t row0, float* x, int64_t ldx,
                  float* probs, int64_t ldp, void* stream);
int gmr_flip_loss_rows(int32_t B, int32_t I, const float* x0, int64_t ld0, const float* z, int64_t ldz,
                       const int32_t* t, const float* tables, int32_t T, float grad_scale, float* dz, int64_t lddz,
                       double* bce_row, double* kl_row, void* stream);
int gmr_flip_total(const double* bce_kl, const float* cl, float w_cl, float* out4, void* stream);
int gmr_layernorm_fwd(int64_t rows, int32_t D, const float* a, int64_t lda, const float* b, int64_t ldb,
                      const uint8_t* keep, int64_t ld_keep, float keep_scale, const float* w, const float* bias,
                      float eps, int32_t gelu, float* y, int64_t ldy, float* s_out, int64_t lds, float* mean,
                      float* rstd, void* stream);
int gmr_layernorm_drop_fwd(int64_t rows, int32_t D, const float* a, int64_t lda, const float* b, int64_t ldb,
                           float p_keep, uint64_t seed, uint64_t step, uint64_t ctr0, uint8_t* keep_out,
                           int64_t ld_keep, float keep_scale, const float* w, const float* bias, float eps,
                           int32_t gelu, float* y, int64_t ldy, float* s_out, int64_t lds, float* mean, float* rstd,
                           void* stream);
int64_t gmr_layernorm_parts_floats(int64_t rows, int32_t D);
int gmr_layernorm_bwd(int64_t rows, int32_t D, const float* s, int64_t lds, const float* mean, const float* rstd,
                      const float* w, const float* bias, int32_t gelu, const float* dy, int64_t lddy, float* dx,
                      int64_t lddx, int32_t accumulate_dx, float* parts, float* dw, float* db,
                      int32_t accumulate_params, void* stream);
int gmr_adaln_fwd(int64_t rows, int32_t D, const float* h0, int64_t ld0, const int32_t* t, int32_t t_const,
                  const float* S, int64_t lds, float* h1, int64_t ld1, void* stream);
int gmr_adaln_bwd(int64_t rows, int32_t D, const float* h0, int64_t ld0, const float* dh1, int64_t ldd,
                  const int32_t* t, const float* S, int64_t lds, float* dh0, int64_t ldo, float* prod, int64_t ldp,
                  void* stream);
int gmr_dropout_f32(int64_t rows, int32_t D, int32_t group, const float* x, int64_t ldx, float p_keep,
                    const uint8_t* mask_in, uint8_t* mask_out, int64_t ldm, uint64_t seed, uint64_t step, int64_t row0,
                    float* y, int64_t ldy, void* stream);
int gmr_xattn_table_f32(int32_t L, int32_t D, int32_t nhead, const float* woc0, const float* bvc0,
                        int64_t layer_stride, float p_keep, float* P, void* stream);
int gmr_xattn_fwd_f32(int64_t rows, int32_t D, int32_t nhead, const float* P, const float* bo, float p_keep,
                      const uint8_t* mask_in, uint8_t* mask_out, int64_t ldm, uint64_t seed, uint64_t step, int64_t row0,
                      float* CA, int64_t ldc, void* stream);
int64_t gmr_xattn_bwd_workspace_floats(int64_t rows, int32_t D, int32_t nhead);
int gmr_xattn_bwd_f32(int64_t rows, int32_t D, int32_t nhead, const float* dCA, int64_t ld, const uint8_t* mask,
                      int64_t ldm, const float* wo, const float* bv, float p_keep, float* g_wo, float* g_bv, float* ws,
                      int64_t ws_floats, void* stream);
int gmr_decoder_layers_fwd_f32(int64_t B, int64_t Bmax, int32_t L, int32_t D, int32_t nhead, const float* slab,
                               const int64_t* offsets, int64_t layer_stride, int32_t train_drop, float p_keep,
                               uint64_t seed, uint64_t step, int64_t row0, int32_t reuse_cav, const float* xP,
                               void* const* bufs, int32_t tile, float* gemm_ws, int64_t gemm_ws_floats, void* stream);
int gmr_time_embedding(int32_t T, int32_t E, float* out, void* stream);
int gmr_silu_f32(int64_t n, const float* x, const float* dy, float* y, void* stream);

int gmr_adam_f32(int64_t n, float* param, const float* grad, float* exp_avg, float* exp_avg_sq, float beta1,
                 float beta2, float eps, float weight_decay, float step_size, float bias_correction2_sqrt,
                 void* stream);

int gmr_frd_loss_fwd_bwd(int32_t B, int64_t n_users, const float* G, int64_t ldg, const float* T, int64_t ldt,
                         const float* V, int64_t ldv, const int32_t* users, const int32_t* pos, const int32_t* neg,
                         float reg_weight, float inv_norm, double* parts_ws, float* loss, float* contrib,
                         int64_t ldc, void* stream);
// ... 213 lines not shown
```

Baseline: 306,000 users/s.

## Filter top-1 denoiser output with bf16-hi GEMM plus exact gather recompute

For the final diffusion posterior step when only the top-1 item is needed, a cheap single-plane bf16 GEMM produces approximate scores. Per-row error bounds from precomputed W2 row norms mark candidate columns that could beat the approximate max, and an exact 3-plane split GEMM recomputes only the gathered candidate columns. This is meant to replace the full fp32-accurate 3-plane GEMM over all items with one cheap pass plus a sparse exact pass. It adds stats kernels, new workspace, and kernel template modes, and relies on the error bounds being conservative to keep the selected index exact.

```diff
diff --git a/generative-multimodal-recommendation_amd/csrc/gemm.hip b/generative-multimodal-recommendation_amd/csrc/gemm.hip
--- a/generative-multimodal-recommendation_amd/csrc/gemm.hip
+++ b/generative-multimodal-recommendation_amd/csrc/gemm.hip
@@ -620,6 +620,30 @@
 
 }
 
+namespace gmr_gemm {
+
+bool top1_plan_ok(int64_t M, int64_t N, int64_t K, int tile) {
+  const Plan p = make_plan(0, 1, M, N, K, tile, 0);
+  return p.mf == 6 && p.bm == 128 && p.bn == 128 && p.splits == 1 && !p.x6p && !p.xpose && x6_top1_supported() &&
+         p.tm * p.tn < (1ll << 31);
+}
+
+void top1_product(int mode, hipStream_t st, int64_t M, int64_t N, int64_t K, const float* A, int64_t lda,
+                  const float* B, int64_t ldb, const float* bias, float slope, float* C, int64_t ldc, const int* cols,
+                  const int* ncols) {
+  Epi e = {};
+  e.kind = GMR_EPI_SCALE_BIAS;
+  e.alpha = 1.f;
+  e.slope = slope;
+  e.bias = bias;
+  const int64_t tm = (M + 127) / 128, tn = (N + 127) / 128;
+  const int64_t kps = (K + BK - 1) / BK * BK;
+  const int tnp = mode == 1 ? (int)tn | (tile_group(tn) << 20) : (int)tn;
+  x6_top1_launch(mode, dim3((unsigned)(tm * tn)), st, M, N, K, A, lda, B, ldb, C, ldc, e, tnp, kps, cols, ncols);
+}
+
+}
+
 extern "C" int32_t gmr_gemm_kernel_kind(int32_t trans_a, int32_t trans_b, int64_t M, int64_t N, int64_t K,
                                         int32_t tile, int32_t split_k, int32_t aligned) {
   if (M <= 0 || N <= 0 || K <= 0) return 0;
diff --git a/generative-multimodal-recommendation_amd/csrc/gemm_impl.h b/generative-multimodal-recommendation_amd/csrc/gemm_impl.h
--- a/generative-multimodal-recommendation_amd/csrc/gemm_impl.h
+++ b/generative-multimodal-recommendation_amd/csrc/gemm_impl.h
@@ -341,6 +341,15 @@
               const float* B, int64_t ldb, float* C, int64_t ldc, const Epi& epi, int tiles_n, int64_t kps, float* ws,
               bool akc = true, bool bkc = true, bool pipe = false);
 
+bool x6_top1_supported();
+void x6_top1_launch(int mode, dim3 grid, hipStream_t st, int64_t M, int64_t N, int64_t K, const float* A, int64_t lda,
+                    const float* B, int64_t ldb, float* C, int64_t ldc, const Epi& epi, int tiles_n, int64_t kps,
+                    const int* cols, const int* ncols);
+bool top1_plan_ok(int64_t M, int64_t N, int64_t K, int tile);
+void top1_product(int mode, hipStream_t st, int64_t M, int64_t N, int64_t K, const float* A, int64_t lda,
+                  const float* B, int64_t ldb, const float* bias, float slope, float* C, int64_t ldc, const int* cols,
+                  const int* ncols);
+
 void x6_transpose(const float* src, int64_t ld_src, int64_t rows, int64_t cols, float* dst, int64_t ld_dst,
                   hipStream_t st);
 
diff --git a/generative-multimodal-recommendation_amd/csrc/gemm_x6.hip b/generative-multimodal-recommendation_amd/csrc/gemm_x6.hip
--- a/generative-multimodal-recommendation_amd/csrc/gemm_x6.hip
+++ b/generative-multimodal-recommendation_amd/csrc/gemm_x6.hip
@@ -67,6 +67,20 @@
   }
 }
 
+template <int R, int NT, int N4>
+__device__ __forceinline__ void x6_store_hi(const float4 (&r)[N4], __bf16* s) {
+#pragma unroll
+  for (int i = 0; i < N4; ++i) {
+    const int idx = threadIdx.x + NT * i;
+    const float v[4] = {r[i].x, r[i].y, r[i].z, r[i].w};
+    const int rr = idx / (BK / 4), k4 = (idx % (BK / 4)) * 4;
+    bf16x4 h;
+#pragma unroll
+    for (int e = 0; e < 4; ++e) h[e] = (__bf16)__builtin_amdgcn_fmed3f(v[e], -0x1.fep127f, 0x1.fep127f);
+    *reinterpret_cast<bf16x4*>(s + rr * BK + (((k4 >> 3) ^ x6_swz(rr)) << 3) + (k4 & 7)) = h;
+  }
+}
+
 template <int R, int NT>
 struct KcTile {
   static constexpr int N4 = R * BK / 4 / NT;
@@ -81,6 +95,14 @@
       const int rr = idx / (BK / 4), k4 = (idx % (BK / 4)) * 4;
       const int64_t row = min(r0 + rr, nrows - 1) - r0;
       off[i] = (int)(row * ld) + k4;
+    }
+  }
+  __device__ __forceinline__ void init_gather(int64_t r0, int64_t nrows, int64_t ld, const int* __restrict__ cols) {
+#pragma unroll
+    for (int i = 0; i < N4; ++i) {
+      const int idx = threadIdx.x + NT * i;
+      const int rr = idx / (BK / 4), k4 = (idx % (BK / 4)) * 4;
+      off[i] = (int)((int64_t)cols[min(r0 + rr, nrows - 1)] * ld) + k4;
     }
   }
   __device__ __forceinline__ void load(const float* __restrict__ base) {
@@ -159,18 +181,22 @@
   }
 }
 
-template <int BM, int BN, int WGM, int WGN, int NBUF, int OCC, int PIPE, bool AKC = true, bool BKC = true>
+template <int BM, int BN, int WGM, int WGN, int NBUF, int OCC, int PIPE, bool AKC = true, bool BKC = true, int MODE = 0>
 __global__ void __launch_bounds__(64 * WGM * WGN, OCC) gemm_x6_kernel(int64_t M, int64_t N, int64_t K,
                                                                 const float* __restrict__ A, int64_t lda,
                                                                 const float* __restrict__ B, int64_t ldb,
                                                                 float* __restrict__ C, int64_t ldc, Epi epi,
                                                                 int tiles_n, int64_t k_per_split,
-                                                                float* __restrict__ ws) {
+                                                                float* __restrict__ ws,
+                                                                const int* __restrict__ gcols,
+                                                                const int* __restrict__ gn) {
   constexpr int NT = 64 * WGM * WGN;
   constexpr int WTM = BM / WGM, WTN = BN / WGN;
   constexpr int TM = WTM / 32, TN = WTN / 32;
   constexpr int APL = BM * BK, BPL = BN * BK;
-  constexpr int STAGE = 3 * (APL + BPL);
+  constexpr int NP = MODE == 1 ? 1 : 3;
+  constexpr int STAGE = NP * (APL + BPL);
+  static_assert(MODE == 0 || (PIPE == 0 && AKC && BKC), "the filter modes: NT operands, the PIPE 0 loop");
   __shared__ __attribute__((aligned(16))) __bf16 smem[NBUF * STAGE];
 
   const int nwg = gridDim.x;
@@ -183,6 +209,13 @@
   const int64_t n0 = (int64_t)tni * BN;
   const int64_t kbeg = (int64_t)blockIdx.z * k_per_split;
   const int64_t kend = min(K, kbeg + k_per_split);
+  int64_t nlist = 0;
+  const int* cl = nullptr;
+  if constexpr (MODE == 2) {
+    nlist = gn[tmi];
+    if (n0 >= nlist) return;
+    cl = gcols + (int64_t)tmi * N;
+  }
 
   const int lane = threadIdx.x & 63;
   const int w = threadIdx.x >> 6;
@@ -198,21 +231,21 @@
       for (int e = 0; e < 16; ++e) acc[i][j][e] = sml[i][j][e] = 0.f;
 
   auto mstep = [&](const __bf16* a_s, int s, auto&& gap) {
-    const __bf16* b_s = a_s + 3 * APL;
-    bf16x8 fb[3][TN];
+    const __bf16* b_s = a_s + NP * APL;
+    bf16x8 fb[NP][TN];
 #pragma unroll
     for (int j = 0; j < TN; ++j) {
       const int row = wn * WTN + j * 32 + l32;
       const int off = row * BK + (((2 * s + h) ^ x6_swz(row)) << 3);
 #pragma unroll
-      for (int p = 0; p < 3; ++p) fb[p][j] = *reinterpret_cast<const bf16x8*>(b_s + p * BPL + off);
-    }
-    bf16x8 fa_[TM][3];
+      for (int p = 0; p < NP; ++p) fb[p][j] = *reinterpret_cast<const bf16x8*>(b_s + p * BPL + off);
+    }
+    bf16x8 fa_[TM][NP];
     auto read_a = [&](int i) {
       const int row = wm * WTM + i * 32 + l32;
       const int off = row * BK + (((2 * s + h) ^ x6_swz(row)) << 3);
 #pragma unroll
-      for (int p = 0; p < 3; ++p) fa_[i][p] = *reinterpret_cast<const bf16x8*>(a_s + p * APL + off);
+      for (int p = 0; p < NP; ++p) fa_[i][p] = *reinterpret_cast<const bf16x8*>(a_s + p * APL + off);
     };
     if constexpr (PIPE == 1) {
 #pragma unroll
@@ -222,7 +255,12 @@
 #pragma unroll
     for (int i = 0; i < TM; ++i) {
       if constexpr (PIPE != 1) read_a(i);
-      const bf16x8(&fa)[3] = fa_[i];
+      const bf16x8(&fa)[NP] = fa_[i];
+      if constexpr (MODE == 1) {
+#pragma unroll
+        for (int j = 0; j < TN; ++j)
+          acc[i][j] = __builtin_amdgcn_mfma_f32_32x32x16_bf16(fa[0], fb[0][j], acc[i][j], 0, 0, 0);
+      } else {
 #pragma unroll
       for (int j = 0; j < TN; ++j) {
         const int g = 6 * (i * TN + j);
@@ -239,6 +277,7 @@
         acc[i][j] = __builtin_amdgcn_mfma_f32_32x32x16_bf16(fa[0], fb[0][j], acc[i][j], 0, 0, 0);
         gap(g + 5);
       }
+      }
     }
   };
 
@@ -247,9 +286,10 @@
   std::conditional_t<AKC, KcTile<BM, NT>, MnTile<BM, NT>> ra;
   std::conditional_t<BKC, KcTile<BN, NT>, MnTile<BN, NT>> rb;
   ra.init(m0, M, lda);
-  rb.init(n0, N, ldb);
+  if constexpr (MODE == 2) rb.init_gather(n0, nlist, ldb, cl);
+  else rb.init(n0, N, ldb);
   const float* a0 = AKC ? A + m0 * lda : A + m0;
-  const float* b0 = BKC ? B + n0 * ldb : B + n0;
+  const float* b0 = MODE == 2 ? B : BKC ? B + n0 * ldb : B + n0;
   const int nk = kend > kbeg ? (int)((kend - kbeg + BK - 1) / BK) : 0;
   const int kl = (int)(kend - kbeg - (int64_t)(nk - 1) * BK);
   auto fetch = [&](int t) {
@@ -274,6 +314,11 @@
     }
   };
   auto store = [&](__bf16* s) {
+    if constexpr (MODE == 1) {
+      x6_store_hi<BM, NT>(ra.r, s);
+      x6_store_hi<BN, NT>(rb.r, s + APL);
+      return;
+    }
     if constexpr (AKC) x6_store<BM, true, NT>(ra.r, s);
     else ra.store(s);
     if constexpr (BKC) x6_store<BN, true, NT>(rb.r, s + 3 * APL);
@@ -391,16 +436,34 @@
     }
   }
 
+  if constexpr (MODE != 1) {
 #pragma unroll
   for (int i = 0; i < TM; ++i)
 #pragma unroll
     for (int j = 0; j < TN; ++j) acc[i][j] += sml[i][j];
-
+  }
+
+  if constexpr (MODE != 0) {
+#pragma unroll
+    for (int i = 0; i < TM; ++i)
+#pragma unroll
+      for (int j = 0; j < TN; ++j) {
+        const int64_t n = n0 + wn * WTN + j * 32 + l32;
+        if (n >= (MODE == 2 ? nlist : N)) continue;
+        const float b = epi.bias ? epi.bias[MODE == 2 ? (int64_t)cl[n] : n] : 0.f;
+#pragma unroll
+        for (int e = 0; e < 16; ++e) {
+          const int64_t m = m0 + wm * WTM + i * 32 + (e & 3) + 8 * (e >> 2) + 4 * h;
+          if (m < M) C[m * ldc + n] = epi_fin(epi, acc[i][j][e], b, 0.f, 0.f, 0.f);
+        }
+      }
+  } else {
   if (!ws && epi_reads_x(epi))
     gemm_epilogue_lds<BM, BN, WGM, WGN, NBUF * 3 * (BM + BN) * BK / 2>(acc, reinterpret_cast<float*>(smem), M, N, C,
                                                                      ldc, epi, m0, n0, ws);
   else
     gemm_epilogue<BM, BN, WGM, WGN, 32>(acc, M, N, C, ldc, epi, m0, n0, ws);
+  }
 }
 
 __global__ void __launch_bounds__(256) x6_transpose_kernel(const float* __restrict__ src, int64_t ld_src,
@@ -476,26 +539,26 @@
     if (!akc || !bkc) {                                                                                            \
       if (akc)                                                                                                     \
         hipLaunchKernelGGL((gemm_x6_kernel<BM_, BN_, WGM_, WGN_, NBUF_, OCC_, 0, true, false>), grid,              \
-                           dim3(64 * WGM_ * WGN_), 0, st, M, N, K, A, lda, B, ldb, C, ldc, epi, tiles_n, kps, ws); \
+                           dim3(64 * WGM_ * WGN_), 0, st, M, N, K, A, lda, B, ldb, C, ldc, epi, tiles_n, kps, ws, nullptr, nullptr); \
       else if (!bkc)                                                                                               \
         hipLaunchKernelGGL((gemm_x6_kernel<BM_, BN_, WGM_, WGN_, NBUF_, OCC_, 0, false, false>), grid,             \
-                           dim3(64 * WGM_ * WGN_), 0, st, M, N, K, A, lda, B, ldb, C, ldc, epi, tiles_n, kps, ws); \
+                           dim3(64 * WGM_ * WGN_), 0, st, M, N, K, A, lda, B, ldb, C, ldc, epi, tiles_n, kps, ws, nullptr, nullptr); \
       else                                                                                                         \
         return -1;                                                                                                 \
       return 0;                                                                                                    \
     }                                                                                                              \
     if (NBUF_ == 2 && pipe)                                                                                        \
       hipLaunchKernelGGL((gemm_x6_kernel<BM_, BN_, WGM_, WGN_, NBUF_, OCC_, NBUF_ - 1>), grid, dim3(64 * WGM_ * WGN_), \
-                         0, st, M, N, K, A, lda, B, ldb, C, ldc, epi, tiles_n, kps, ws);                           \
+                         0, st, M, N, K, A, lda, B, ldb, C, ldc, epi, tiles_n, kps, ws, nullptr, nullptr);                           \
     else                                                                                                           \
       hipLaunchKernelGGL((gemm_x6_kernel<BM_, BN_, WGM_, WGN_, NBUF_, OCC_, 0>), grid, dim3(64 * WGM_ * WGN_), 0,   \
-                         st, M, N, K, A, lda, B, ldb, C, ldc, epi, tiles_n, kps, ws);                              \
+                         st, M, N, K, A, lda, B, ldb, C, ldc, epi, tiles_n, kps, ws, nullptr, nullptr);                              \
     return 0;                                                                                                      \
   }
   if (bm == 64 && bn == 64 && (!akc || !bkc)) return -1;
   if (bm == 64 && bn == 64 && x6_ring()) {
     hipLaunchKernelGGL((gemm_x6_kernel<64, 64, 2, 2, 2, 3, 2>), grid, dim3(256), 0, st, M, N, K, A, lda, B, ldb, C,
-                       ldc, epi, tiles_n, kps, ws);
+                       ldc, epi, tiles_n, kps, ws, nullptr, nullptr);
     return 0;
   }
   if (bm == 64 && bn == 64) GMR_X6(64, 64, 2, 2, 2, 3)
@@ -511,4 +574,17 @@
   return -1;
 }
 
-}
+bool x6_top1_supported() { return x6_pipe() != 1 && x6_nb128() == 0; }
+
+void x6_top1_launch(int mode, dim3 grid, hipStream_t st, int64_t M, int64_t N, int64_t K, const float* A, int64_t lda,
+                    const float* B, int64_t ldb, float* C, int64_t ldc, const Epi& epi, int tiles_n, int64_t kps,
+                    const int* cols, const int* ncols) {
+  if (mode == 1)
+    hipLaunchKernelGGL((gemm_x6_kernel<128, 128, 2, 2, 2, 3, 0, true, true, 1>), grid, dim3(256), 0, st, M, N, K, A,
+                       lda, B, ldb, C, ldc, epi, tiles_n, kps, nullptr, nullptr, nullptr);
+  else
+    hipLaunchKernelGGL((gemm_x6_kernel<128, 128, 2, 2, 1, 2, 0, true, true, 2>), grid, dim3(256), 0, st, M, N, K, A,
+                       lda, B, ldb, C, ldc, epi, tiles_n, kps, nullptr, cols, ncols);
+}
+
+}
diff --git a/generative-multimodal-recommendation_amd/csrc/top1_filter.hip b/generative-multimodal-recommendation_amd/csrc/top1_filter.hip
--- /dev/null
+++ b/generative-multimodal-recommendation_amd/csrc/top1_filter.hip
@@ -0,0 +1,204 @@
+#include <math.h>
+
+#include "gemm_impl.h"
+
+namespace {
+
+constexpr int T1_THREADS = 256;
+constexpr int T1_STAGE_COLS = 12288;
+constexpr float T1_UP = 1.f + 0x1p-20f;
+
+__device__ __forceinline__ uint32_t fkey(float f) {
+  uint32_t u = __float_as_uint(f);
+  return (u & 0x80000000u) ? ~u : (u | 0x80000000u);
+}
+
+__device__ __forceinline__ bool finite_f(float x) { return fabsf(x) <= 3.402823466e38f; }
+
+__device__ __forceinline__ void stat_acc(const float* __restrict__ x, int64_t k, double& ss, double& es) {
+  for (int64_t c = threadIdx.x; c < k; c += T1_THREADS) {
+    const float v = x[c];
+    const float hi = (float)(__bf16)__builtin_amdgcn_fmed3f(v, -0x1.fep127f, 0x1.fep127f);
+    const double d = (double)v - (double)hi;
+    ss += (double)v * (double)v;
+    es += d * d;
+  }
+}
+
+__device__ __forceinline__ double block_sum_d(double v, double* red) {
+  v = gmr::wave_sum_d(v);
+  __syncthreads();
+  if ((threadIdx.x & 63) == 0) red[threadIdx.x >> 6] = v;
+  __syncthreads();
+  return (red[0] + red[1]) + (red[2] + red[3]);
+}
+
+__global__ void __launch_bounds__(T1_THREADS) top1_row_stats_kernel(int64_t k, const float* __restrict__ X, int64_t ld,
+                                                                    float2* __restrict__ st) {
+  __shared__ double red[4];
+  const int64_t r = blockIdx.x;
+  double ss = 0.0, es = 0.0;
+  stat_acc(X + r * ld, k, ss, es);
+  ss = block_sum_d(ss, red);
+  es = block_sum_d(es, red);
+  if (threadIdx.x == 0)
+    st[r] = make_float2((float)(sqrt(ss) * (1.0 + 0x1p-8)) * T1_UP, (float)sqrt(es) * T1_UP);
+}
+
+template <bool STAGED>
+__global__ void __launch_bounds__(T1_THREADS) top1_mark_kernel(int64_t N, int64_t K, const float* __restrict__ XA,
+                                                               int64_t ldx, const float* __restrict__ H, int64_t ldh,
+                                                               const float2* __restrict__ wst, float c1abs, double acc,
+                                                               unsigned char* __restrict__ flags,
+                                                               int* __restrict__ row_marks) {
+  extern __shared__ float s_row[];
+  __shared__ double red[4];
+  __shared__ float red_f[4];
+  __shared__ int red_i[4];
+  const int64_t row = blockIdx.x;
+  const float* p = XA + row * ldx;
+  double ss = 0.0, es = 0.0;
+  stat_acc(H + row * ldh, K, ss, es);
+  ss = block_sum_d(ss, red);
+  es = block_sum_d(es, red);
+  const double hn = sqrt(ss) * (1.0 + 0x1p-8);
+  const float fa = (float)((double)c1abs * (sqrt(es) + acc * hn) * (1.0 + 0x1p-18));
+  const float fb = (float)((double)c1abs * hn * (1.0 + 0x1p-18));
+  auto radius = [&](float a, float2 w) { return fmaf(fa, w.x, fb * w.y) + 0x1p-21f * fabsf(a); };
+
+  float lb = -INFINITY;
+  int bad = 0;
+  for (int64_t j = threadIdx.x; j < N; j += T1_THREADS) {
+    const float a = p[j];
+    if (STAGED) s_row[j] = a;
+    const float d = radius(a, wst[j]);
+    bad |= !(finite_f(a) && finite_f(d));
+    lb = fmaxf(lb, a - d);
+  }
+  lb = gmr::wave_max(lb);
+  bad = __any(bad);
+  if ((threadIdx.x & 63) == 0) red_f[threadIdx.x >> 6] = lb, red_i[threadIdx.x >> 6] = bad;
+  __syncthreads();
+  lb = fmaxf(fmaxf(red_f[0], red_f[1]), fmaxf(red_f[2], red_f[3]));
+  bad = red_i[0] | red_i[1] | red_i[2] | red_i[3];
+
+  unsigned char* f = flags + (row / 128) * N;
+  int cnt = 0;
+  for (int64_t j = threadIdx.x; j < N; j += T1_THREADS) {
+    const float a = STAGED ? s_row[j] : p[j];
+    if (bad || a + radius(a, wst[j]) >= lb) {
+      f[j] = 1;
+      ++cnt;
+    }
+  }
+  if (row_marks) {
+#pragma unroll
+    for (int m = 32; m >= 1; m >>= 1) cnt += __shfl_xor(cnt, m);
+    __syncthreads();
+    if ((threadIdx.x & 63) == 0) red_i[threadIdx.x >> 6] = cnt;
+    __syncthreads();
+    if (threadIdx.x == 0) row_marks[row] = red_i[0] + red_i[1] + red_i[2] + red_i[3];
+  }
+}
+
+__global__ void __launch_bounds__(T1_THREADS) top1_compact_kernel(int64_t N, const unsigned char* __restrict__ flags,
+                                                                  int* __restrict__ cols, int* __restrict__ ncols) {
+  __shared__ int scan[T1_THREADS];
+  const int64_t b = blockIdx.x;
+  const unsigned char* f = flags + b * N;
+  const int t = threadIdx.x;
+  const int64_t chunk = (N + T1_THREADS - 1) / T1_THREADS;
+  const int64_t c0 = min(N, t * chunk), c1 = min(N, c0 + chunk);
+  int n = 0;
+  for (int64_t j = c0; j < c1; ++j) n += f[j] != 0;
+  scan[t] = n;
+  __syncthreads();
+  for (int off = 1; off < T1_THREADS; off <<= 1) {
+    const int a = t >= off ? scan[t - off] : 0;
+    __syncthreads();
+    scan[t] += a;
+    __syncthreads();
+  }
+  int64_t o = b * N + scan[t] - n;
+  for (int64_t j = c0; j < c1; ++j)
+    if (f[j]) cols[o++] = (int)j;
+  if (t == T1_THREADS - 1) ncols[b] = scan[t];
+}
+
+__global__ void __launch_bounds__(T1_THREADS) top1_select_kernel(int64_t M, int64_t N, const float* __restrict__ S,
+                                                                 int64_t ld, const int* __restrict__ cols,
+                                                                 const int* __restrict__ ncols,
+                                                                 int* __restrict__ out_idx, int64_t ld_idx) {
+  const int64_t row = (int64_t)blockIdx.x * (T1_THREADS / 64) + (threadIdx.x >> 6);
+  if (row >= M) return;
+  const int64_t b = row / 128;
+  const int n = ncols[b];
+  const int* cl = cols + b * N;
+  const float* p = S + row * ld;
+  unsigned long long best = ~0ull;
+  for (int q = threadIdx.x & 63; q < n; q += 64) {
+    const unsigned long long e = ((unsigned long long)(~fkey(p[q])) << 32) | (uint32_t)cl[q];
+    best = e < best ? e : best;
+  }
+#pragma unroll
+  for (int m = 32; m >= 1; m >>= 1) {
+    const unsigned long long o = __shfl_xor(best, m);
+    best = o < best ? o : best;
+  }
+  if ((threadIdx.x & 63) == 0) out_idx[row * ld_idx] = (int)(uint32_t)(best & 0xFFFFFFFFull);
+}
+
+}
+
+extern "C" int gmr_top1_row_stats_f32(int64_t n_rows, int64_t n_cols, const float* x, int64_t ld, float* stats,
+                                      void* stream) {
+  GMR_ARG(x && stats && n_rows > 0 && n_cols > 0 && ld >= n_cols && n_rows < (1ll << 31), "bad args");
+  GMR_ARG(((uintptr_t)stats & 7) == 0, "stats must be 8-byte aligned");
+  hipLaunchKernelGGL(top1_row_stats_kernel, dim3((unsigned)n_rows), dim3(T1_THREADS), 0, (hipStream_t)stream, n_cols,
+                     x, ld, reinterpret_cast<float2*>(stats));
+  GMR_LAUNCHED();
+  return GMR_OK;
+}
+
+extern "C" int32_t gmr_top1_filter_ok(int64_t M, int64_t N, int64_t K, int32_t tile, const float* h, int64_t ldh,
+                                      const float* W, int64_t ldw) {
+  if (M <= 0 || N <= 0 || K <= 0 || !h || !W) return 0;
+  if (((uintptr_t)h & 15) || ((uintptr_t)W & 15) || ldh % 4 || ldw % 4 || ldh < K || ldw < K) return 0;
+  if (M >= (1ll << 31) || N * ldw >= (1ll << 31)) return 0;
+  return gmr_gemm::top1_plan_ok(M, N, K, tile) ? 1 : 0;
+}
+
+extern "C" int gmr_top1_filter_f32(int64_t M, int64_t N, int64_t K, const float* h, int64_t ldh, const float* W,
+                                   int64_t ldw, const float* bias, float c1, const float* w_stats, int32_t tile,
+                                   float* approx, int64_t ld_approx, float* exact, int64_t ld_exact, uint8_t* flags,
+                                   int32_t* cols, int32_t* ncols, int32_t* row_marks, int32_t* out_idx, int64_t ld_idx,
+                                   void* stream) {
+  GMR_ARG(h && W && bias && w_stats && approx && exact && flags && cols && ncols && out_idx, "null argument");
+  GMR_ARG(ld_approx >= N && ld_exact >= N && ld_idx >= 1, "leading dimension too small");
+  GMR_ARG(((uintptr_t)w_stats & 7) == 0, "w_stats must be 8-byte aligned");
+  GMR_ARG(gmr_top1_filter_ok(M, N, K, tile, h, ldh, W, ldw),
+          "needs 16-byte aligned operands and the split-bf16 128^2 unsplit plan (gmr_top1_filter_ok)");
+  hipStream_t st = (hipStream_t)stream;
+  const int64_t nb = (M + 127) / 128;
+  const hipError_t e = hipMemsetAsync(flags, 0, (size_t)(nb * N), st);
+  if (e != hipSuccess) return gmr::hip_status(__func__, e);
+  gmr_gemm::top1_product(1, st, M, N, K, h, ldh, W, ldw, bias, c1, approx, ld_approx, nullptr, nullptr);
+  GMR_LAUNCHED();
+  const double acc = 2.0 * (double)(K + 4) * 0x1p-23;
+  const float2* wst = reinterpret_cast<const float2*>(w_stats);
+  if (N <= T1_STAGE_COLS)
+    hipLaunchKernelGGL(top1_mark_kernel<true>, dim3((unsigned)M), dim3(T1_THREADS), sizeof(float) * (size_t)N, st, N,
+                       K, approx, ld_approx, h, ldh, wst, fabsf(c1), acc, flags, row_marks);
+  else
+    hipLaunchKernelGGL(top1_mark_kernel<false>, dim3((unsigned)M), dim3(T1_THREADS), 0, st, N, K, approx, ld_approx, h,
+                       ldh, wst, fabsf(c1), acc, flags, row_marks);
+  GMR_LAUNCHED();
+  hipLaunchKernelGGL(top1_compact_kernel, dim3((unsigned)nb), dim3(T1_THREADS), 0, st, N, flags, cols, ncols);
+  GMR_LAUNCHED();
+  gmr_gemm::top1_product(2, st, M, N, K, h, ldh, W, ldw, bias, c1, exact, ld_exact, cols, ncols);
+  GMR_LAUNCHED();
+  hipLaunchKernelGGL(top1_select_kernel, dim3((unsigned)((M + T1_THREADS / 64 - 1) / (T1_THREADS / 64))),
+                     dim3(T1_THREADS), 0, st, M, N, exact, ld_exact, cols, ncols, out_idx, ld_idx);
+  GMR_LAUNCHED();
+  return GMR_OK;
+}
diff --git a/generative-multimodal-recommendation_amd/gmr/_lib.py b/generative-multimodal-recommendation_amd/gmr/_lib.py
--- a/generative-multimodal-recommendation_amd/gmr/_lib.py
+++ b/generative-multimodal-recommendation_amd/gmr/_lib.py
@@ -112,6 +112,10 @@
     "gmr_diff_time_bwd": (I32, [I32, I32, I32, P, P, P, P, I64, I64, P, P, P, P, I32, P]),
     "gmr_mask_scores_f32": (I32, [I64, P, P, P, I64, F32, P]),
     "gmr_topk_rows_f32": (I32, [I64, I64, P, I64, I32, P, I64, P, P]),
+    "gmr_top1_row_stats_f32": (I32, [I64, I64, P, I64, P, P]),
+    "gmr_top1_filter_ok": (I32, [I64, I64, I64, I32, P, I64, P, I64]),
+    "gmr_top1_filter_f32": (I32, [I64, I64, I64, P, I64, P, I64, P, F32, P, I32, P, I64, P, I64, P, P, P, P, P, I64,
+                                  P]),
     "gmr_score_topk_f32": (I32, [I64, P, P, I64, I64, P, I64, I64, P, P, F32, I32, P, I64, P, P]),
     "gmr_score_topk_x6": (I32, [I64, P, P, I64, I64, P, I64, I64, I64, P, P, F32, I32, P, I64, P, P]),
     "gmr_eval_metrics_partials": (I64, [I64]),
diff --git a/generative-multimodal-recommendation_amd/gmr/denoise.py b/generative-multimodal-recommendation_amd/gmr/denoise.py
--- a/generative-multimodal-recommendation_amd/gmr/denoise.py
+++ b/generative-multimodal-recommendation_amd/gmr/denoise.py
@@ -14,6 +14,7 @@
 
 
 PSAMPLE_FOLD = os.environ.get("GMR_PSAMPLE_FOLD", "1") != "0"
+REBUILD_FILTER = os.environ.get("GMR_REBUILD_FILTER", "1") != "0"
 
 
 class _Linear(nn.Module):
@@ -84,7 +85,19 @@
                   self._w1t.stride(0), stream())
         if PSAMPLE_FOLD:
             self.refresh_fold()
+        self._w2st_ok = False
+        if REBUILD_FILTER:
+            self.w2_stats()
         return self._w1t
+
+    def w2_stats(self):
+        if getattr(self, "_w2st", None) is None:
+            self._w2st = torch.empty((self.I, 2), device=self.device)
+            self._w2st_ok = False
+        if not getattr(self, "_w2st_ok", False):
+            K.top1_row_stats(self.slab.view("W2"), self._w2st)
+            self._w2st_ok = True
+        return self._w2st
 
     def refresh_fold(self):
         H = self.H
@@ -96,7 +109,7 @@
         K.gemm(self.slab.view("b2")[None, :], self.W1x(), v, trans_b=True)
         return self._fold
 
-    def p_sample_fold(self, users, user_ptr, user_items, EB, c1, c2, x, a, h):
+    def p_sample_fold(self, users, user_ptr, user_items, EB, c1, c2, x, a, h, last=True):
         T = len(c1)
         if c2[0] != 0.0:
             raise ValueError("p_sample_fold needs c2[0] == 0 (the posterior mean at t = 0 is the x0 prediction)")
@@ -107,7 +120,7 @@
         for i in range(T - 1, 0, -1):
             K.gemm(h, P, a, trans_b=True, epi=K.EPI_POSTERIOR, bias=v[0], aux=a, slope=c1[i], beta=c2[i])
             _lib.call("gmr_tanh_bias_f32", B, H, ptr(a), a.stride(0), ptr(EB[i - 1]), ptr(h), h.stride(0), stream())
-        return self.posterior_step(h, x, c1[0], 0.0)
+        return self.posterior_step(h, x, c1[0], 0.0) if last else h
 
     def hidden_sparse(self, users, user_ptr, user_items, h, eb_row):
         _lib.call("gmr_diff_sparse_hidden", users.numel(), self.H, ptr(users), ptr(user_ptr), ptr(user_items),
@@ -134,6 +147,13 @@
                    slope=c1, beta=c2)
         return x
 
+    def top1_applies(self, h):
+        return K.top1_filter_ok(h, self.slab.view("W2"))
+
+    def posterior_top1(self, h, approx, exact, work, out_idx, c1):
+        return K.top1_filter(h, self.slab.view("W2"), self.slab.view("b2"), c1, self.w2_stats(), approx, exact, work,
+                             out_idx)
+
     def slab_head_words(self):
         return self.slab.offsets["W2"]
 
diff --git a/generative-multimodal-recommendation_amd/gmr/diffmm.py b/generative-multimodal-recommendation_amd/gmr/diffmm.py
--- a/generative-multimodal-recommendation_amd/gmr/diffmm.py
+++ b/generative-multimodal-recommendation_amd/gmr/diffmm.py
@@ -577,14 +577,25 @@
         xi = x[:, :I]
         c1 = [float(np.float32(c)) for c in self.tables["c1"]]
         c2 = [float(np.float32(c)) for c in self.tables["c2"]]
+        top1 = (dn.REBUILD_FILTER and k == 1 and x_out is None and out_topk is not None and c2[0] == 0.0
+                and den.top1_applies(h))
         if dn.PSAMPLE_FOLD:
-            den.p_sample_fold(users, self.user_ptr, self.user_items, EB, c1, c2, xi, w["a"][:B], h)
+            den.p_sample_fold(users, self.user_ptr, self.user_items, EB, c1, c2, xi, w["a"][:B], h, last=not top1)
         for i in reversed(range(T)) if not dn.PSAMPLE_FOLD else ():
             if i == T - 1:
                 den.hidden_sparse(users, self.user_ptr, self.user_items, h, EB[i])
             else:
                 den.hidden(xi, h, EB, t_const=i)
-            den.posterior_step(h, xi, float(np.float32(self.tables["c1"][i])), float(np.float32(self.tables["c2"][i])))
+            if i > 0 or not top1:
+                den.posterior_step(h, xi, float(np.float32(self.tables["c1"][i])),
+                                   float(np.float32(self.tables["c2"][i])))
+        if top1:
+            fw = w.get("top1")
+            if fw is None or fw["M"] < B:
+                fw = w["top1"] = K.top1_filter_work(w["B"], I, self.device)
+            den.posterior_top1(h, xi, w["out"][:B, :I], fw, out_topk[users_lo:users_hi], c1[0])
+            self.top1_filter_calls = getattr(self, "top1_filter_calls", 0) + 1
+            return None
         if x_out is not None:
             x_out.copy_(xi)
         if out_topk is not None:
diff --git a/generative-multimodal-recommendation_amd/gmr/kernels.py b/generative-multimodal-recommendation_amd/gmr/kernels.py
--- a/generative-multimodal-recommendation_amd/gmr/kernels.py
+++ b/generative-multimodal-recommendation_amd/gmr/kernels.py
@@ -584,6 +584,36 @@
     return out_idx
 
 
+def top1_row_stats(W, stats):
+    n, k = W.shape
+    _lib.call("gmr_top1_row_stats_f32", n, k, ptr(W), _ld(W), ptr(stats), stream())
+    return stats
+
+
+def top1_filter_ok(h, W, tile=0):
+    M, Kd = h.shape
+    return bool(_lib.load().gmr_top1_filter_ok(M, W.shape[0], Kd, tile | GEMM_TILE_FLAGS, ptr(h), _ld(h), ptr(W),
+                                               _ld(W)))
+
+
+def top1_filter_work(M, N, device):
+    nb = (M + 127) // 128
+    return {"M": M, "N": N, "flags": torch.empty((nb, N), dtype=torch.uint8, device=device),
+            "cols": torch.empty((nb, N), dtype=torch.int32, device=device),
+            "ncols": torch.empty(nb, dtype=torch.int32, device=device)}
+
+
+def top1_filter(h, W, bias, c1, w_stats, approx, exact, work, out_idx, tile=0, row_marks=None):
+    M, Kd = h.shape
+    N = W.shape[0]
+    if work["M"] < M or work["N"] != N:
+        raise ValueError("top1_filter: scratch too small (top1_filter_work)")
+    _lib.call("gmr_top1_filter_f32", M, N, Kd, ptr(h), _ld(h), ptr(W), _ld(W), ptr(bias), float(c1), ptr(w_stats),
+              tile | GEMM_TILE_FLAGS, ptr(approx), _ld(approx), ptr(exact), _ld(exact), ptr(work["flags"]),
+              ptr(work["cols"]), ptr(work["ncols"]), ptr(row_marks), ptr(out_idx), _ld(out_idx), stream())
+    return out_idx
+
+
 EVAL_X6 = os.environ.get("GMR_EVAL_X6", "0") != "0"
 _item_planes = {}
 
diff --git a/include/gmr.h b/include/gmr.h
--- a/include/gmr.h
+++ b/include/gmr.h
@@ -255,6 +255,13 @@
                         void* stream);
 int gmr_topk_rows_f32(int64_t n_rows, int64_t n_cols, const float* scores, int64_t ld, int32_t k, int32_t* out_idx,
                       int64_t ld_idx, float* out_val, void* stream);
+int gmr_top1_row_stats_f32(int64_t n_rows, int64_t n_cols, const float* x, int64_t ld, float* stats, void* stream);
+int32_t gmr_top1_filter_ok(int64_t M, int64_t N, int64_t K, int32_t tile, const float* h, int64_t ldh, const float* W,
+                           int64_t ldw);
+int gmr_top1_filter_f32(int64_t M, int64_t N, int64_t K, const float* h, int64_t ldh, const float* W, int64_t ldw,
+                        const float* bias, float c1, const float* w_stats, int32_t tile, float* approx,
+                        int64_t ld_approx, float* exact, int64_t ld_exact, uint8_t* flags, int32_t* cols,
+                        int32_t* ncols, int32_t* row_marks, int32_t* out_idx, int64_t ld_idx, void* stream);
 int gmr_score_topk_f32(int64_t n_rows, const int32_t* users, const float* user_table, int64_t ld_user, int64_t n_items,
                        const float* item_table, int64_t ld_item, int64_t dim, const int64_t* mask_ptr,
                        const int32_t* mask_cols, float fill, int32_t k, int32_t* out_idx, int64_t ld_idx,
```

Result: no change. 310,300 users/s (median of 4 runs) (+1.4%).
